# karfly/learnable-triangulation-pytorch

Measured on AMD Instinct MI355X. Metric: multi-view samples/sec (4-view vol-softmax forward), higher is better.
Workload: dtype bf16; 1 GPU; BASELINE config 2: volumetric-softmax forward, 4 views 384x384, 64^3 voxel cube, ResNet-152, random-init weights; per_gpu_batch=64, global_batch=64, parallelism=batch-sharded replicas x1, no data-path collective, hip_graph=True, self_launched=False

## Files before the change

### include/lt_hip.h

```cpp
#ifndef LT_HIP_H
#define LT_HIP_H

#include <stddef.h>
#include <stdint.h>

#ifdef __cplusplus
extern "C" {
#endif

#define LT_ABI_VERSION 1

enum { LT_F32 = 0, LT_BF16 = 1,
       LT_FP8 = 2  };
enum { LT_OK = 0, LT_ERR_INVALID = -1, LT_ERR_UNSUPPORTED = -2, LT_ERR_LAUNCH = -3 };

enum { LT_AGG_SUM = 0, LT_AGG_MAX = 1, LT_AGG_SOFTMAX = 2, LT_AGG_CONF = 3,
       LT_AGG_CONF_NORM = 4  };

enum {
    LT_EPI_RELU_PRE = 1,
    LT_EPI_RELU_POST = 2,
    LT_EPI_STORE_F32 = 4,
    LT_EPI_SIGMOID = 8,
    LT_EPI_RES_F32 = 64,
    LT_BN_FROZEN = 32,
    LT_BN_Y_BF16 = 128,
    LT_ACT_BF16 = 256
};

const char* lt_last_error(void);
int lt_abi_version(void);
int lt_device_info(int* cu_count, int* lds_per_cu, char* arch, int arch_len);

#define LT_CONV_MAX_PHASES 8

typedef struct lt_conv_phase {
    const void* weight;
    const int32_t* taps;
    int32_t ntaps;
    int32_t out_off[3];
    const void* weight_frag;
    int32_t weight_frag_layout;
} lt_conv_phase;

typedef struct lt_conv_desc {
    int32_t dtype;
    int32_t N, D, H, W, Cin;
    int32_t Do, Ho, Wo;
    int32_t stride[3], pad[3];
    int32_t OD, OH, OW;
    int32_t out_stride[3];
    int32_t Cout, ldc;
    int32_t cout_pad, k_pad;
    int32_t nphase;
    int32_t flags;
    int32_t tile;
    int32_t stages;
    lt_conv_phase phase[LT_CONV_MAX_PHASES];
} lt_conv_desc;

int lt_conv_pack_weights(const void* weight, int32_t cout_pad, int32_t k_pad, void* packed, void* stream);
int lt_conv_pack_weights_t32(const void* weight, int32_t cout_pad, int32_t k_pad, int32_t cin, int32_t ntaps, void* packed,
                             void* stream);
int lt_conv_pack_weights32(const void* weight, int32_t cout_pad, int32_t k_pad, void* packed, void* stream);

enum { LT_TILE_AUTO = 0,
       LT_TILE_128x128 = 1, LT_TILE_128x64 = 2, LT_TILE_256x32 = 3, LT_TILE_256x16 = 4, LT_TILE_64x64 = 5,
       LT_TILE2_128x128 = 11, LT_TILE2_128x64 = 12, LT_TILE2_256x32 = 13, LT_TILE2_256x16 = 14, LT_TILE2_64x64 = 15,
       LT_TILE_HALO = 20,
       LT_TILE3_288 = 30,
       LT_TILE_DIRECT = 99  };

int lt_conv_fwd(const lt_conv_desc* desc, const void* x, const float* bias, const float* scale, const float* shift,
                const void* residual, void* y, void* stream);
typedef struct lt_conv_skip {
    const void* x;
    int32_t cin;
    const void* weight_frag;
} lt_conv_skip;
int lt_conv_skip_fwd(const lt_conv_desc* desc, const void* x, const float* bias, const float* scale, const float* shift,
                     const lt_conv_skip* skip, void* y, void* stream);
typedef struct lt_conv_cat2 {
    const void* x;
    int32_t cin, H, W, stride;
} lt_conv_cat2;
int lt_conv_cat2_fwd(const lt_conv_desc* desc, const void* x, const lt_conv_cat2* second, const float* bias, const float* scale, const float* shift,
                     const void* residual, void* y, void* stream);
int lt_conv_cout_pad(int32_t cout);
int32_t lt_conv_chunk_samples(int32_t N, int64_t per_sample);

typedef struct lt_wshape {
    int32_t nd;
    int64_t s[5];
} lt_wshape;
int lt_sel_conv_skip(int32_t dtype, const int32_t x[5], const lt_wshape* w, const int32_t skip_x[5], const lt_wshape* skip_w);
int lt_sel_conv_cat2(int32_t dtype, const int32_t t2[5], const lt_wshape* w_expand, const int32_t x[5], const lt_wshape* w_down, int32_t stride_down);
int lt_sel_splitk_slices(const lt_conv_desc* d, const lt_wshape* w, int32_t transposed);
int lt_sel_bottleneck(int32_t dtype, const int32_t x[5], const lt_wshape w[3], const int32_t strides[3]);
int lt_sel_bottleneck_ds(int32_t dtype, const int32_t x[5], const lt_wshape w[3], const int32_t strides[3], const lt_wshape* w_down, int32_t stride_down);
int lt_sel_expand_reduce(int32_t dtype, const int32_t t2[5], const int32_t res[5], const lt_wshape* w_expand, const lt_wshape* w_reduce);
int lt_sel_stem_pool(int32_t dtype, const int32_t x[5], const lt_wshape* w, int32_t stride, int32_t pad, const int32_t pool[3]);
int lt_sel_pwchain(int32_t dtype, const int32_t x[5], int32_t nlayers, const lt_wshape* w);
int lt_sel_frag_layout(const lt_conv_desc* d, const lt_wshape* w, int32_t transposed, int32_t has_residual);

int lt_maxpool_fwd(int32_t dtype, const void* x, void* y, int32_t N, int32_t D, int32_t H, int32_t W, int32_t C,
                   const int32_t k[3], const int32_t s[3], const int32_t p[3], void* stream);

int lt_global_avgpool(int32_t dtype, const void* x, void* y, int32_t N, int32_t HW, int32_t C, void* stream);

int lt_nchw_to_nhwc(int32_t dtype, const float* x, void* y, int32_t N, int32_t C, int32_t HW, int32_t c_pad, void* stream);
int lt_nhwc_to_nchw_f32(int32_t dtype, const void* x, float* y, int32_t N, int32_t C, int32_t HW, int32_t ld, void* stream);

int lt_splitk_reduce(int32_t dtype, const float* partial, int32_t S, int64_t N, int64_t rows_per_sample, int32_t C, const float* bias,
                     const float* scale, const float* shift, const void* residual, void* y, int32_t flags, void* stream);

int lt_coord_volumes(const float* pos, const float* center, const float* rot, float step, int32_t B, int32_t V,
                     int32_t cmu_transfer, float* coords, void* stream);
int lt_rotate_points(const float* x, const float* rot, float* y, int64_t n, void* stream);

int lt_unproject_fwd(int32_t dtype, const void* feats, const float* proj, const float* coords, const float* conf,
                     void* out, int32_t B, int32_t NV, int32_t C, int32_t h, int32_t w, int32_t v0, int32_t v1,
                     int32_t v2, int32_t agg, void* stream);
int lt_unproject_grid_fwd(int32_t dtype, const void* feats, const float* proj, const float* pos, const float* center, const float* rot,
                          float step, int32_t cmu_transfer, float* coords_out, const float* conf, void* out, int32_t B, int32_t NV,
                          int32_t C, int32_t h, int32_t w, int32_t V, int32_t agg, void* stream);
int lt_unproject_masked_fwd(int32_t dtype, const void* feats, const float* proj, const float* coords, const float* conf, const uint8_t* view_mask,
                            void* out, int32_t B, int32_t NV, int32_t C, int32_t h, int32_t w, int32_t v0, int32_t v1, int32_t v2, int32_t agg,
                            void* stream);
int lt_unproject_grid_masked_fwd(int32_t dtype, const void* feats, const float* proj, const float* pos, const float* center, const float* rot,
                                 float step, int32_t cmu_transfer, float* coords_out, const float* conf, const uint8_t* view_mask, void* out,
                                 int32_t B, int32_t NV, int32_t C, int32_t h, int32_t w, int32_t V, int32_t agg, void* stream);
enum { LT_KIND_MPII = 0, LT_KIND_COCO = 1 };
int lt_cuboid_from_keypoints(const float* keypoints_3d, int32_t B, int32_t J, int32_t kind, double cuboid_side, float* pos, float* center,
                             void* stream);

size_t lt_softargmax3d_workspace(int32_t B, int32_t J, int64_t nvox);
int lt_softargmax3d_fwd(const float* logits, const float* coords, float mult, int32_t softmax, int32_t channels_last,
                        int32_t ld, float* kp, float* probs, int32_t B, int32_t J, int64_t nvox, void* workspace,
                        void* stream);

int lt_softargmax2d_fwd(const float* heatmaps, float mult, int32_t softmax, float* coords, float* probs, int32_t NJ,
                        int32_t h, int32_t w, void* stream);
int lt_softargmax2d_bwd(const float* probs, const float* coords, const float* grad_coords, float mult, int32_t softmax, float* grad_heatmaps,
                        int32_t NJ, int32_t h, int32_t w, void* stream);
int lt_triangulate_dlt_bwd(const float* proj, const float* points, const float* conf, const float* grad_out, float* grad_points, float* grad_conf,
                           int32_t B, int32_t NV, int32_t J, void* stream);

size_t lt_unproject_bwd_workspace(int32_t B, int32_t NV, int32_t C, int32_t v0, int32_t v1, int32_t v2);
int lt_unproject_bwd(int32_t dtype, const void* feats, const float* proj, const float* coords, const float* conf, const float* grad_out,
                     float* grad_feats, float* grad_conf, int32_t B, int32_t NV, int32_t C, int32_t h, int32_t w, int32_t v0, int32_t v1,
                     int32_t v2, int32_t agg, void* workspace, size_t workspace_bytes, void* stream);
int lt_softargmax3d_bwd(const float* probs, const float* coords, const float* kp, const float* grad_kp, const int32_t* gp_idx,
                        const float* gp_val, float multiplier, int32_t softmax, int32_t channels_last, float* grad_logits, int32_t B,
                        int32_t J, int64_t nvox, void* stream);
int lt_softargmax3d_bwd_dense(const float* probs, const float* coords, const float* kp, const float* grad_kp, const int32_t* gp_idx,
                              const float* gp_val, const float* gp_dense, float* workspace_bj, float multiplier, int32_t softmax,
                              int32_t channels_last, float* grad_logits, int32_t B, int32_t J, int64_t nvox, void* stream);
int lt_volumetric_ce_fwd(const float* coords, const float* probs, const float* keypoints_gt, const float* validity, float* terms,
                         int32_t* idx, float* grad_val, int32_t B, int32_t J, int64_t nvox, void* stream);
size_t lt_bn_stats_workspace(int64_t rows, int32_t C);
int lt_bn_stats_fwd(int32_t dtype, const void* x, int64_t rows, int32_t C, float* mean, float* var, float* running_mean,
                    float* running_var, float momentum, void* workspace, void* stream);

int lt_bn_act_fwd(const void* y , const float* mean, const float* var, const float* gamma, const float* beta, const void* residual, void* z,
                  void* z_bf16 , int64_t rows, int32_t C, float eps,
                  int32_t flags, void* stream);
size_t lt_bn_act_bwd_workspace(int64_t rows, int32_t C);
int lt_bn_act_bwd(const void* dz, const void* y , const void* residual, const float* mean, const float* var, const float* gamma, const float* beta,
                  void* dy, void* dy_bf16 , float* dgamma, float* dbeta, void* dres, int32_t accumulate_res,
                  int64_t rows, int32_t C, float eps, int32_t flags, void* workspace, void* stream);
int lt_act_bwd(const void* dz, const void* z, const void* residual, void* dy, void* dres, int32_t accumulate_res, int64_t total, int32_t flags,
               void* stream);
size_t lt_channel_sum_workspace(int64_t rows, int32_t C);
int lt_channel_sum(const float* x, int64_t rows, int32_t C, float* out, int32_t accumulate, void* workspace, void* stream);
int lt_channel_sum_dt(int32_t dtype, const void* x, int64_t rows, int32_t C, float* out, int32_t accumulate, void* workspace, void* stream);
int lt_maxpool_bwd(const float* x, const float* dy, float* dx, int32_t N, int32_t D, int32_t H, int32_t W, int32_t C, const int32_t k[3],
                   const int32_t s[3], const int32_t p[3], void* stream);
int lt_maxpool_bwd_dt(int32_t dtype, const void* x, const void* dy, void* dx, int32_t N, int32_t D, int32_t H, int32_t W, int32_t C, const int32_t k[3],
                      const int32_t s[3], const int32_t p[3], void* stream);
size_t lt_conv_wgrad_workspace(int64_t rows, int32_t cout_pad, int32_t k_pad);
int lt_conv_wgrad(const float* dy, const float* x, const int32_t* taps, float* dw, int32_t N, int32_t D, int32_t H, int32_t W, int32_t Cin, int32_t Do,
                  int32_t Ho, int32_t Wo, const int32_t stride[3], const int32_t pad[3], int32_t Cout, int32_t ldy, int32_t cout_pad, int32_t k_pad,
// ... 26 lines not shown
int lt_quant_fp8_dt(int32_t dtype, const void* x, void* q, int64_t n, const float* amax, float* scale_out, void* stream);
int lt_gather_f32_fp8(const float* src, const int32_t* idx, void* q, int64_t n, const float* amax, float* scale_out, void* stream);
int lt_scale_product(float* dst, int32_t n, const float* a, const float* b, void* stream);
int lt_gather_f32_multi(const void* jobs, int32_t njobs, int32_t total_blocks, void* stream);
int lt_adam_step_multi(const void* jobs, int32_t njobs, int32_t total_blocks, double beta1, double beta2, float eps, float weight_decay, int32_t step,
                       void* stream);
int lt_adam_step(float* param, const float* grad, float* exp_avg, float* exp_avg_sq, int64_t n, float lr, double beta1, double beta2, float eps,
                 float weight_decay, int32_t step, void* stream);

int lt_triangulate_dlt(const float* proj, const float* points, const float* conf, float* out, int32_t B, int32_t NV,
                       int32_t J, void* stream);
int lt_alg_tail_fwd(const float* keypoints_hm, const float* conf_raw, int32_t ld_conf, const float* proj, float scale_x, float scale_y,
                    float* keypoints_2d, float* confidences, float* keypoints_3d, int32_t B, int32_t NV, int32_t J, void* stream);
int lt_alg_tail_masked_fwd(const float* keypoints_hm, const float* conf_raw, int32_t ld_conf, const float* proj, float scale_x, float scale_y,
                           const uint8_t* view_mask, float* keypoints_2d, float* confidences, float* keypoints_3d, int32_t B, int32_t NV,
                           int32_t J, void* stream);

int lt_heatmap_argmax_nchw_f32(const float* heatmaps, int32_t ld, float* heatmaps_nchw, int64_t* indices, int64_t* keypoints,
                               int32_t N, int32_t J, int32_t h, int32_t w, int32_t image_h, int32_t image_w, void* stream);
int lt_triangulate_ransac(const float* proj, const int64_t* points, const int32_t* pairs, int32_t n_iters, double eps, int32_t direct_opt,
                          float* out_kp3d, uint8_t* out_inliers, int32_t B, int32_t NV, int32_t J, void* stream);

int lt_crop_resize_u8(const uint8_t* src, int64_t src_bytes, const int64_t* desc, const int64_t* desc_host, int32_t N, int32_t H, int32_t W,
                      const float* lut, float* out, void* stream);

int lt_undistort_crop_resize_u8(const uint8_t* src, int64_t src_bytes, const int64_t* desc, const int64_t* desc_host, const int16_t* maps,
                                int64_t maps_bytes, int32_t N, int32_t H, int32_t W, const float* lut, float* out, void* stream);

#define LT_PWCHAIN_MAX 3
typedef struct {
    int32_t dtype;
    int32_t nlayers;
    int64_t rows;
    int32_t cin;
    int32_t ldy;
    int32_t cout[LT_PWCHAIN_MAX];
    int32_t k_pad[LT_PWCHAIN_MAX];
    int32_t flags[LT_PWCHAIN_MAX];
    const void* weight[LT_PWCHAIN_MAX];
    const float* bias[LT_PWCHAIN_MAX];
    const float* scale[LT_PWCHAIN_MAX];
    const float* shift[LT_PWCHAIN_MAX];
    int64_t plane;
} lt_pwchain_desc;
int lt_pwchain_fwd(const lt_pwchain_desc* desc, const void* x, void* y, void* stream);

typedef struct {
    int32_t dtype;
    int32_t N, H, W;
    int32_t Cin, Cout;
    const void* weight;
    const float* bias;
    const float* scale;
    const float* shift;
    int32_t x_layout;
} lt_stem_desc;
size_t lt_stem_packed_bytes(void);
int lt_stem_pack_weights(const void* weight, int32_t k_pad, void* packed, void* stream);
int lt_stem_pool_fwd(const lt_stem_desc* desc, const void* x, void* y, void* stream);

typedef struct {
    int32_t dtype;
    int32_t N, H, W;
    int32_t C, P;
    const void* weight[3];
    const float* bias[3];
    const float* scale[3];
    const float* shift[3];
} lt_bneck_desc;
int lt_bottleneck_fwd(const lt_bneck_desc* desc, const void* x, void* y, void* stream);

typedef struct {
    int32_t dtype;
    int32_t N, H, W;
    int32_t Cin, P, C;
    const void* weight[4];
    const float* scale[4];
    const float* shift[4];
} lt_bneck_ds_desc;
int lt_bottleneck_ds_fwd(const lt_bneck_ds_desc* desc, const void* x, void* y, void* stream);

typedef struct {
    int32_t dtype;
    int32_t C, P;
    int64_t M;
    const void* weight[2];
    const float* scale[2];
    const float* shift[2];
    const float* consts;
} lt_xr_desc;
int lt_expand_reduce_fwd(const lt_xr_desc* desc, const void* t2, const void* residual, void* y, void* t1_next, void* stream);

int lt_graph_begin(void* stream);
int lt_graph_end(void* stream, void** graph_exec_out);
int lt_graph_launch(void* graph_exec, void* stream);
int lt_graph_destroy(void* graph_exec);
int lt_event_create(void** ev_out);
int lt_event_record(void* ev, void* stream);
int lt_event_elapsed_ms(void* ev_start, void* ev_stop, float* ms_out);
int lt_event_destroy(void* ev);

typedef struct lt_plan lt_plan;
typedef struct lt_named_tensor {
    const char* name;
    const float* data;
    int32_t ndim;
    int64_t shape[5];
} lt_named_tensor;
typedef struct lt_vol_plan_config {
    int32_t dtype;
    int32_t num_layers;
    int32_t style_caffe;
    int32_t num_joints;
    int32_t B, NV, H, W;
    int32_t volume_size;
    double cuboid_side;
    double volume_multiplier;
    int32_t volume_softmax;
    int32_t aggregation;
    int32_t transfer_cmu_to_human36m;
    int32_t use_graph;
} lt_vol_plan_config;
typedef struct lt_plan_info_t {
    int32_t launches;
    int32_t heatmap_h, heatmap_w;
    double flops;
    int64_t bytes_allocated;
    int32_t n_expand_reduce, n_bottleneck, n_bottleneck_ds, n_conv_cat2, n_conv2d_halo, n_pwchain, n_stem_pool, n_splitk, n_conv_skip;
    int32_t graph_captured;
    const float* logits;
    int32_t logits_planar;
} lt_plan_info_t;
int lt_plan_create_vol(const lt_vol_plan_config* cfg, const lt_named_tensor* weights, int32_t nweights, lt_plan** plan_out);
int lt_plan_forward_vol(lt_plan* plan, const float* images, const double* K_host, const double* R_host, const double* t_host, const double* base_points_host,
                        const double* rot_host, float* keypoints_3d, float* volumes, float* features, float* coord_volumes, float* vol_confidences, void* stream);
enum { LT_MODEL_ALG = 1, LT_MODEL_RANSAC = 2 };
typedef struct lt_alg_plan_config {
    int32_t model;
    int32_t dtype;
    int32_t num_layers;
    int32_t style_caffe;
    int32_t num_joints;
    int32_t B, NV, H, W;
    int32_t use_confidences;
    int32_t heatmap_softmax;
    double heatmap_multiplier;
    int32_t direct_optimization;
    double reprojection_error_epsilon;
    int32_t use_graph;
} lt_alg_plan_config;
int lt_plan_create_alg(const lt_alg_plan_config* cfg, const lt_named_tensor* weights, int32_t nweights, lt_plan** plan_out);
int lt_plan_forward_alg(lt_plan* plan, const float* images, const float* proj, float* keypoints_3d, void* keypoints_2d, float* heatmaps,
                        float* confidences, void* stream);
typedef struct lt_cascade_plan_config {
    lt_alg_plan_config alg;
    lt_vol_plan_config vol;
    int32_t kind;
} lt_cascade_plan_config;
int lt_plan_create_cascade(const lt_cascade_plan_config* cfg, const lt_named_tensor* alg_weights, int32_t n_alg, const lt_named_tensor* vol_weights,
                           int32_t n_vol, lt_plan** plan_out);
int lt_plan_forward_cascade(lt_plan* plan, const float* images, const double* K_host, const double* R_host, const double* t_host, const double* rot_host,
                            float* keypoints_3d, float* alg_keypoints_3d, float* base_points, float* volumes, float* features, float* coord_volumes,
                            float* vol_confidences, void* stream);
int lt_plan_set_view_mask(lt_plan* plan, const uint8_t* mask_host);
int lt_plan_info(const lt_plan* plan, lt_plan_info_t* info);
void lt_plan_destroy(lt_plan* plan);
// ... 6 lines not shown
```

### learnable-triangulation-pytorch_amd/csrc/bneck.hip

```cpp
#include <stdlib.h>

#include <type_traits>

#include "wave_prims.h"

using namespace lt;

namespace {

__device__ uint4 g_zero_page_b[2];

#ifdef LT_BNECK_TRACE
#define LT_BNECK_TRACE_WG 4096
__device__ unsigned long long g_bneck_trace[LT_BNECK_TRACE_WG * 4 * 8];
#define BN_STAMP(k)                                                                                                  \
    do {                                                                                                             \
        if (blockIdx.x < LT_BNECK_TRACE_WG && lane == 0) g_bneck_trace[(blockIdx.x * 4 + wave) * 8 + (k)] = clock64(); \
    } while (0)
#else
#define BN_STAMP(k)
#endif

struct BneckArgs {
    const bf16_t* x;
    bf16_t* y;
    const bf16_t* w1;
    const bf16_t* w2;
    const bf16_t* w3;
    const float* bias[3];
    const float* scale[3];
    const float* shift[3];
    int N, H, W, tiles_x, tiles_y;
};

template <int NK1, int AHEAD, int D>
constexpr int bneck_after(int ks) {
    int total = 0, last = 0;
    for (int k = 0; k < D && k < NK1; ++k) { total += 2; if (k == ks) last = total; }
    for (int k = 0; k < AHEAD && k < NK1; ++k) { total += 3; if (k == ks && total > last) last = total; }
    for (int s = 0; s < ks; ++s) {
        if (s + D < NK1) { total += 2; if (s + D == ks && total > last) last = total; }
        if (s + AHEAD < NK1) { total += 3; if (s + AHEAD == ks && total > last) last = total; }
    }
    return total - last;
}

template <int C, int P, int NSTR, int NHELD>
__global__ __launch_bounds__(256, 2) void bneck_kernel(const BneckArgs a) {
    typedef bf16_t T;
    constexpr int TH = 8, TW = 16, HPI = TW + 2, HROWS = (TH + 2) * HPI;
    constexpr int NPB = 4;
    constexpr int NCB = P / 32, NOB = C / 32, G2 = P / 16, NK1 = C / 32;
    constexpr int RB = 2 * P, NSL = P / 8;
    constexpr int T1_BYTES = HROWS * RB;
    constexpr int STAGE = HROWS * 64;
    constexpr int NT1 = T1_BYTES / STAGE, NST = NT1 + NSTR;
    constexpr int T2_OFF = T1_BYTES;
    constexpr int AHEAD = NST - 1 < NK1 ? NST - 1 : NK1;
    constexpr int NPB1 = NCB == 4 ? 6 : 3, NPB2 = NCB == 4 ? 4 : 2, NOBW = NOB / 4;
    static_assert(NCB == 2 || NCB == 4, "bottleneck width 64 or 128");
    static_assert(T1_BYTES % STAGE == 0, "t1 is a whole number of ring stages");
    static_assert(NPB * 32 * RB <= (NSTR - 1) * STAGE + 192 * 64, "t2 fits behind t1");
    static_assert(NK1 % 2 == 0 && NHELD <= NOBW && NHELD <= 2, "K steps / held residual blocks");
    static_assert(T1_BYTES % 256 == 0 && STAGE % 256 == 0, "the XOR / bank arguments assume 256-byte aligned regions");
    auto fsw = [](int hp) -> int { return NSL == 16 ? (hp & 15) : ((hp >> 1) & 7); };

    extern __shared__ __attribute__((aligned(1024))) unsigned char smem[];
    const unsigned lds0 = (unsigned)(size_t)(lptr_t)smem;
    unsigned long long zp_bits = (unsigned long long)(size_t)g_zero_page_b;
    asm volatile("" : "+s"(zp_bits));
    const void* const zero_page = (const void*)(size_t)zp_bits;

    const int t = threadIdx.x, lane = t & 63;
    const int wave = __builtin_amdgcn_readfirstlane(t >> 6);
    int lin = blockIdx.x;
    {
        const int nb = gridDim.x, q = nb >> 3, r = nb & 7, xcd = lin & 7, j = lin >> 3;
        lin = (xcd < r ? xcd * (q + 1) : r * (q + 1) + (xcd - r) * q) + j;
    }
    const int tpi = a.tiles_x * a.tiles_y;
    const int img = lin / tpi, rem = lin - img * tpi;
    const int ty = rem / a.tiles_x, tx = rem - ty * a.tiles_x;
    const int y0 = ty * TH - 1, x0 = tx * TW - 1;
    const T* __restrict__ x = a.x;

    const int n31 = lane & 31, hk = lane >> 5;
    const int cb = NCB == 4 ? wave : (wave & 1);
    const int whalf = NCB == 4 ? 0 : (wave >> 1);
    const int prr = n31 >> 4, pcc = ((n31 & 15) - 2 * prr) & 15;

    uint4 held[NHELD > 0 ? NHELD : 1][NPB][2];

    float4 cst12, cst3;
    {
        const int l = lane & 31, arr = l >> 3, i4 = l & 7;
        const float* t12 = arr == 0 ? a.scale[0] : arr == 1 ? a.shift[0] : arr == 2 ? a.scale[1] : a.shift[1];
        cst12 = *(const float4*)(t12 + 32 * cb + 4 * i4);
        const int f = (4 * lane) % (NOBW * 64), q = f >> 6, which = (f >> 5) & 1, c = f & 31;
        cst3 = *(const float4*)((which ? a.shift[2] : a.scale[2]) + 32 * (wave + 4 * q) + c);
    }
    auto cget = [&](const float4& tb, int f) -> float {
        const float v = (f & 3) == 0 ? tb.x : (f & 3) == 1 ? tb.y : (f & 3) == 2 ? tb.z : tb.w;
        return __int_as_float(__builtin_amdgcn_readlane(__float_as_int(v), f >> 2));
    };
    auto csel = [&](const float4& tb, int base, int e) -> float {
        const float lo = cget(tb, base + 16 * (e >> 3) + (e & 7)), hi = cget(tb, base + 16 * (e >> 3) + 8 + (e & 7));
        return hk ? hi : lo;
    };

    BN_STAMP(0);
    {
#ifndef LT_BNECK_ABL_SEG128
        const int prow = lane >> 2;
#endif
#ifdef LT_BNECK_ABL_SEG128
        const int prow = lane >> 3;
        const int kvlog = lane & 7;
#elif defined(LT_BNECK_ABL_NOSWZ)
        const int kvlog = lane & 3;
#else
        const int kvlog = (lane & 3) ^ swz64(prow);
#endif
        int dbase[3];
        bool dact[3];
#pragma unroll
        for (int i = 0; i < 3; ++i) {
            const int hp = 16 * (wave + 4 * i) + prow;
            const int hr = hp / HPI, hc = hp - hr * HPI;
            const int iy = y0 + hr, ix = x0 + hc;
            const bool ok = (hp < HROWS) & ((unsigned)iy < (unsigned)a.H) & ((unsigned)ix < (unsigned)a.W);
            dbase[i] = ok ? ((img * a.H + iy) * a.W + ix) * C + kvlog * 8 : -1;
// ... 35 lines not shown
                for (int j = 0; j < 2; ++j)
                    dst[pb][j] = *(const uint4*)((lptr_t)(size_t)(lds0 + stage_base + hpc * 64 + (((2 * j + hk) ^ swz64(hpc)) << 4)));
            }
        };

        f32x16 acc[NPB1];
#pragma unroll
        for (int i = 0; i < NPB1; ++i)
#pragma unroll
            for (int e = 0; e < 16; ++e) acc[i][e] = 0.f;

        static_for<0, DA>([&](auto kc) { loadA(decltype(kc)::value, fa[decltype(kc)::value]); });
#pragma unroll
        for (int s = 0; s < AHEAD; ++s)
            static_for<0, 3>([&](auto ic) { issue_piece(s, s * STAGE, ic); });

        static_for<0, NK1>([&](auto kc) {
            constexpr int ks = decltype(kc)::value, R = ks % NFA;
            constexpr unsigned rbuf = (ks % NST) * STAGE, wbuf = ((ks + AHEAD) % NST) * STAGE;
            wait_vmcnt<bneck_after<NK1, AHEAD, DA>(ks)>();
            asm volatile("s_waitcnt lgkmcnt(0)\n\ts_barrier" ::: "memory");
            frag_ready(fa[R][0]);
            frag_ready(fa[R][1]);
            if constexpr (ks + DA < NK1) loadA(ks + DA, fa[(ks + DA) % NFA]);
            if constexpr (ks + AHEAD < NK1) static_for<0, 3>([&](auto ic) { issue_piece(ks + AHEAD, wbuf, ic); });
            if constexpr (NHELD > 0 && ks < 4) { if (ks == wave) capture(rbuf, held[0]); }
            if constexpr (NHELD > 1 && ks >= 4 && ks < 8) { if (ks == wave + 4) capture(rbuf, held[NHELD > 1 ? 1 : 0]); }
            const unsigned rb = lds0 + rbuf + hb0 * 2048;
#ifndef LT_BNECK_ABL_NOMMA1
            V16 b0[NPB1], b1[NPB1];
#pragma unroll
            for (int i = 0; i < NPB1; ++i) b0[i].u = *(const uint4*)((lptr_t)(size_t)(rb + fo0 + i * 2048));
            __builtin_amdgcn_sched_barrier(0);
#pragma unroll
            for (int i = 0; i < NPB1; ++i) b1[i].u = *(const uint4*)((lptr_t)(size_t)(rb + fo1 + i * 2048));
#pragma unroll
            for (int i = 0; i < NPB1; ++i) acc[i] = __builtin_amdgcn_mfma_f32_32x32x16_bf16(fa[R][0].h, b0[i].h, acc[i], 0, 0, 0);
            __builtin_amdgcn_sched_barrier(0);
#pragma unroll
            for (int i = 0; i < NPB1; ++i) acc[i] = __builtin_amdgcn_mfma_f32_32x32x16_bf16(fa[R][1].h, b1[i].h, acc[i], 0, 0, 0);
            __builtin_amdgcn_sched_barrier(0);
#else
            acc[0][0] += fa[R][0].f[0] + fa[R][1].f[0];
#endif
        });
        asm volatile("s_waitcnt vmcnt(0)\n\ts_waitcnt lgkmcnt(0)\n\ts_barrier" ::: "memory");
        BN_STAMP(1);

        float esc[16], esf[16];
#pragma unroll
        for (int e = 0; e < 16; ++e) {
            esc[e] = csel(cst12, 0, e);
            esf[e] = csel(cst12, 32, e);
        }
        if (a.bias[0]) {
#pragma unroll
            for (int e = 0; e < 16; ++e) esf[e] = a.bias[0][32 * cb + 16 * (e >> 3) + 8 * hk + (e & 7)] * esc[e] + esf[e];
        }
#pragma unroll
        for (int i = 0; i < NPB1; ++i) {
            const int hp = 32 * (hb0 + i) + n31;
            const int hr = hp / HPI, hc = hp - hr * HPI;
            const int iy = y0 + hr, ix = x0 + hc;
            const bool inimg = ((unsigned)iy < (unsigned)a.H) & ((unsigned)ix < (unsigned)a.W);
            if (hp < HROWS) {
#pragma unroll
                for (int q = 0; q < 2; ++q) {
                    unsigned o[4];
#pragma unroll
                    for (int d = 0; d < 4; ++d) {
                        const int e = 8 * q + 2 * d;
                        const float v0 = fmaxf(acc[i][e] * esc[e] + esf[e], 0.f), v1 = fmaxf(acc[i][e + 1] * esc[e + 1] + esf[e + 1], 0.f);
                        o[d] = inimg ? pack_bf16x2(v0, v1) : 0u;
                    }
                    const int slot = (4 * cb + 2 * q + hk) ^ fsw(hp);
                    *(uint4*)((lptr_t)(size_t)(lds0 + hp * RB + slot * 16)) = make_uint4(o[0], o[1], o[2], o[3]);
                }
            }
        }
    }
    __syncthreads();
    BN_STAMP(2);

    constexpr int NU3 = NOBW * G2, WD3 = G2 < 6 ? G2 : 6;
    int poff[NPB];
#pragma unroll
    for (int pb = 0; pb < NPB; ++pb)
        poff[pb] = ((img * a.H + ty * TH + 2 * pb + prr) * a.W + tx * TW + pcc) * C + 8 * hk;
    const T* wl3 = a.w3 + (size_t)lane * 8;
    auto load_w3 = [&](int u) -> V16 {
        const int q = u / G2, g = u - q * G2;
        V16 v;
        v.u = *(const uint4*)(wl3 + ((size_t)g * NOB + wave + 4 * q) * 512);
        return v;
    };
    V16 wf3[WD3 + 1];
    uint4 rq[2][NPB][2];
    auto load_res = [&](int q, uint4 (&dst)[NPB][2]) {
        const int ob = wave + 4 * q;
#pragma unroll
        for (int pb = 0; pb < NPB; ++pb)
#pragma unroll
            for (int j = 0; j < 2; ++j) dst[pb][j] = *(const uint4*)(x + poff[pb] + 32 * ob + 16 * j);
    };

    {
        const int pb0 = NCB == 4 ? 0 : 2 * whalf;
        const int bn = prr * HPI + pcc + 2 * HPI * pb0;
        unsigned am[16];
#pragma unroll
        for (int m = 0; m < 16; ++m) am[m] = lds0 + bn * RB + ((hk ^ fsw(bn + m)) << 4);
        const T* wl = a.w2 + ((size_t)cb * 64 + lane) * 8;
        auto load_w = [&](int u) -> V16 {
            V16 v;
            v.u = *(const uint4*)(wl + (size_t)u * NCB * 512);
            return v;
        };
        constexpr int NU = 9 * G2, WD = 6;
        V16 wf[WD + 1];
#pragma unroll
        for (int u = 0; u < WD; ++u) wf[u] = load_w(u);
        f32x16 acc[NPB2];
#pragma unroll
        for (int i = 0; i < NPB2; ++i)
#pragma unroll
            for (int e = 0; e < 16; ++e) acc[i][e] = 0.f;
        V16 xa[2][NPB2];
        auto load_x = [&](auto uc, V16 (&dst)[NPB2]) {
            constexpr int u = decltype(uc)::value;
            constexpr int tap = u / G2, g = u % G2, dy = tap / 3, dx = tap % 3;
            static_for<0, NPB2>([&](auto ic) {
                constexpr int i = decltype(ic)::value;
                constexpr int TT = dy * HPI + dx + 2 * HPI * i;
                const unsigned ad = am[TT & 15] ^ (g << 5);
                dst[i].u = *(const uint4*)((lptr_t)(size_t)(ad + TT * RB));
            });
        };
        load_x(std::integral_constant<int, 0>{}, xa[0]);
        static_for<0, NU>([&](auto uc) {
            constexpr int u = decltype(uc)::value;
            if constexpr (u + WD < NU) wf[(u + WD) % (WD + 1)] = load_w(u + WD);
            if constexpr (u + 1 < NU) load_x(std::integral_constant<int, u + 1>{}, xa[(u + 1) & 1]);
#pragma unroll
            for (int i = 0; i < NPB2; ++i)
                acc[i] = __builtin_amdgcn_mfma_f32_32x32x16_bf16(wf[u % (WD + 1)].h, xa[u & 1][i].h, acc[i], 0, 0, 0);
            __builtin_amdgcn_sched_barrier(0);
        });
        BN_STAMP(3);
#pragma unroll
        for (int u = 0; u < WD3; ++u) wf3[u] = load_w3(u);
        if constexpr (NHELD < NOBW) load_res(NHELD, rq[0]);
        __builtin_amdgcn_sched_barrier(0);

        float esc[16], esf[16];
#pragma unroll
        for (int e = 0; e < 16; ++e) {
            esc[e] = csel(cst12, 64, e);
            esf[e] = csel(cst12, 96, e);
        }
        if (a.bias[1]) {
#pragma unroll
            for (int e = 0; e < 16; ++e) esf[e] = a.bias[1][32 * cb + 16 * (e >> 3) + 8 * hk + (e & 7)] * esc[e] + esf[e];
        }
#pragma unroll
        for (int i = 0; i < NPB2; ++i) {
            const int px = 32 * (pb0 + i) + n31;
#pragma unroll
            for (int q = 0; q < 2; ++q) {
                unsigned o[4];
#pragma unroll
                for (int d = 0; d < 4; ++d) {
                    const int e = 8 * q + 2 * d;
                    o[d] = pack_bf16x2(fmaxf(acc[i][e] * esc[e] + esf[e], 0.f), fmaxf(acc[i][e + 1] * esc[e + 1] + esf[e + 1], 0.f));
                }
                const int slot = (4 * cb + 2 * q + hk) ^ fsw(n31);
                *(uint4*)((lptr_t)(size_t)(lds0 + T2_OFF + px * RB + slot * 16)) = make_uint4(o[0], o[1], o[2], o[3]);
            }
        }
    }
    __syncthreads();
    BN_STAMP(4);

    {
        const unsigned a2 = lds0 + T2_OFF + n31 * RB + ((hk ^ fsw(n31)) << 4);
        f32x16 acc[NPB];
        static_for<0, NU3>([&](auto uc) {
            constexpr int u = decltype(uc)::value;
            constexpr int q = u / G2, g = u % G2;
            const int ob = wave + 4 * q;
            if constexpr (g == 0) {
#pragma unroll
                for (int pb = 0; pb < NPB; ++pb)
#pragma unroll
                    for (int e = 0; e < 16; ++e) acc[pb][e] = 0.f;
            }
            if constexpr (g == G2 - WD3 && q + 1 < NOBW && q + 1 > NHELD) load_res(q + 1, rq[(q + 1 - NHELD) & 1]);
            if constexpr (u + WD3 < NU3) wf3[(u + WD3) % (WD3 + 1)] = load_w3(u + WD3);
            V16 xb[NPB];
#pragma unroll
            for (int pb = 0; pb < NPB; ++pb) xb[pb].u = *(const uint4*)((lptr_t)(size_t)((a2 ^ (g << 5)) + pb * 32 * RB));
#pragma unroll
            for (int pb = 0; pb < NPB; ++pb)
                acc[pb] = __builtin_amdgcn_mfma_f32_32x32x16_bf16(wf3[u % (WD3 + 1)].h, xb[pb].h, acc[pb], 0, 0, 0);
            __builtin_amdgcn_sched_barrier(0);
            if constexpr (g == G2 - 1) {
#pragma unroll
                for (int j = 0; j < 2; ++j) {
                    float esc[8], esf[8];
#pragma unroll
                    for (int e = 0; e < 8; ++e) {
                        esc[e] = csel(cst3, 64 * q, 8 * j + e);
                        esf[e] = csel(cst3, 64 * q + 32, 8 * j + e);
                    }
                    if (a.bias[2]) {
#pragma unroll
                        for (int e = 0; e < 8; ++e) esf[e] = a.bias[2][32 * ob + 16 * j + 8 * hk + e] * esc[e] + esf[e];
                    }
#pragma unroll
                    for (int pb = 0; pb < NPB; ++pb) {
                        uint4 rv;
                        if constexpr (q < NHELD) rv = held[q < NHELD ? q : 0][pb][j];
                        else rv = rq[(q - NHELD) & 1][pb][j];
                        const unsigned rr[4] = {rv.x, rv.y, rv.z, rv.w};
                        unsigned o[4];
#pragma unroll
                        for (int d = 0; d < 4; ++d) {
                            const int e = 2 * d;
                            const float v0 = fmaxf(acc[pb][8 * j + e] * esc[e] + esf[e] + __uint_as_float(rr[d] << 16), 0.f);
                            const float v1 = fmaxf(acc[pb][8 * j + e + 1] * esc[e + 1] + esf[e + 1] + __uint_as_float(rr[d] & 0xffff0000u), 0.f);
                            o[d] = pack_bf16x2(v0, v1);
                        }
                        *(uint4*)(a.y + poff[pb] + 32 * ob + 16 * j) = make_uint4(o[0], o[1], o[2], o[3]);
                    }
                }
            }
        });
    }
    BN_STAMP(5);
}

template <int C, int P, int NSTR, int NHELD>
int launch_bneck(const BneckArgs& a, hipStream_t s) {
    constexpr int RB = 2 * P;
    constexpr int lds = 180 * RB + (NSTR - 1) * 180 * 64 + 192 * 64;
    static_assert(lds <= 80 * 1024, "two workgroups per CU");
    auto kern = bneck_kernel<C, P, NSTR, NHELD>;
    LT_OPT_IN_LDS(kern, lds);
    const long long nblk = (long long)a.N * a.tiles_x * a.tiles_y;
    hipLaunchKernelGGL(kern, dim3((unsigned)nblk), dim3(256), lds, s, a);
    LT_CHECK_LAUNCH("lt_bottleneck_fwd");
    return LT_OK;
}


struct BneckDsArgs {
    const bf16_t* x;
    bf16_t* y;
    const bf16_t* w1;
    const bf16_t* w2;
    const bf16_t* w3;
    const bf16_t* wd;
    const float* scale[4];
    const float* shift[4];
    int N, H, W, tiles_x, tiles_y;
};

template <int CIN, int P, int C>
__global__ __launch_bounds__(256, 2) void bneck_ds_kernel(const BneckDsArgs a) {
    typedef bf16_t T;
    constexpr int TH = 8, TW = 16, HPI = TW + 2, HROWS = (TH + 2) * HPI;
    constexpr int NPB = 4;
    constexpr int NCB = P / 32, NOB = C / 32, G2 = P / 16, GD = CIN / 16, NK1 = CIN / 32;
    constexpr int RB = 2 * P, NSL = P / 8;
    constexpr int T1_BYTES = HROWS * RB, STAGE = HROWS * 64;
    constexpr int XS_OFF = T1_BYTES, T2_OFF = XS_OFF + NK1 * STAGE;
    constexpr int NPB1 = 3, NPB2 = 2, NOBW = NOB / 4;
    static_assert(CIN == 64 && P == 64 && C == 256, "the first block of ResNet layer1");
    static_assert(NCB == 2 && NSL == 8 && NOBW == 2, "wave roles below");
    static_assert(XS_OFF % 256 == 0 && T2_OFF % 256 == 0, "the XOR / bank arguments assume 256-byte aligned regions");
    auto fsw = [](int hp) -> int { return (hp >> 1) & 7; };

    extern __shared__ __attribute__((aligned(1024))) unsigned char smem[];
    const unsigned lds0 = (unsigned)(size_t)(lptr_t)smem;
    unsigned long long zp_bits = (unsigned long long)(size_t)g_zero_page_b;
    asm volatile("" : "+s"(zp_bits));
    const void* const zero_page = (const void*)(size_t)zp_bits;

    const int t = threadIdx.x, lane = t & 63;
    const int wave = __builtin_amdgcn_readfirstlane(t >> 6);
    int lin = blockIdx.x;
    {
        const int nb = gridDim.x, q = nb >> 3, r = nb & 7, xcd = lin & 7, j = lin >> 3;
        lin = (xcd < r ? xcd * (q + 1) : r * (q + 1) + (xcd - r) * q) + j;
    }
    const int tpi = a.tiles_x * a.tiles_y;
    const int img = lin / tpi, rem = lin - img * tpi;
    const int ty = rem / a.tiles_x, tx = rem - ty * a.tiles_x;
    const int y0 = ty * TH - 1, x0 = tx * TW - 1;
    const T* __restrict__ x = a.x;

    const int n31 = lane & 31, hk = lane >> 5;
    const int cb = wave & 1, whalf = wave >> 1;
    const int prr = n31 >> 4, pcc = ((n31 & 15) - 2 * prr) & 15;

    float4 cst12, cst3;
    {
        const int l = lane & 31, arr = l >> 3, i4 = l & 7;
        const float* t12 = arr == 0 ? a.scale[0] : arr == 1 ? a.shift[0] : arr == 2 ? a.scale[1] : a.shift[1];
        cst12 = *(const float4*)(t12 + 32 * cb + 4 * i4);
        const int f = 4 * lane, q = f >> 7, which = (f >> 5) & 3, c = f & 31;
        const float* t3 = which == 0 ? a.scale[2] : which == 1 ? a.shift[2] : which == 2 ? a.scale[3] : a.shift[3];
        cst3 = *(const float4*)(t3 + 32 * (wave + 4 * q) + c);
    }
    auto cget = [&](const float4& tb, int f) -> float {
        const float v = (f & 3) == 0 ? tb.x : (f & 3) == 1 ? tb.y : (f & 3) == 2 ? tb.z : tb.w;
        return __int_as_float(__builtin_amdgcn_readlane(__float_as_int(v), f >> 2));
    };
    auto csel = [&](const float4& tb, int base, int e) -> float {
        const float lo = cget(tb, base + 16 * (e >> 3) + (e & 7)), hi = cget(tb, base + 16 * (e >> 3) + 8 + (e & 7));
        return hk ? hi : lo;
    };
// ... 205 lines not shown
            if constexpr (k == NUQ - 1) {
#pragma unroll
                for (int j = 0; j < 2; ++j) {
                    float esc[8], esf[8], dsc[8], dsf[8];
#pragma unroll
                    for (int e = 0; e < 8; ++e) {
                        esc[e] = csel(cst3, 128 * q, 8 * j + e);
                        esf[e] = csel(cst3, 128 * q + 32, 8 * j + e);
                        dsc[e] = csel(cst3, 128 * q + 64, 8 * j + e);
                        dsf[e] = csel(cst3, 128 * q + 96, 8 * j + e);
                    }
#pragma unroll
                    for (int pb = 0; pb < NPB; ++pb) {
                        unsigned o[4];
#pragma unroll
                        for (int d = 0; d < 4; ++d) {
                            const int e = 2 * d;
                            const float r0 = accd[pb][8 * j + e] * dsc[e] + dsf[e], r1 = accd[pb][8 * j + e + 1] * dsc[e + 1] + dsf[e + 1];
                            const float v0 = fmaxf(acc[pb][8 * j + e] * esc[e] + esf[e] + r0, 0.f);
                            const float v1 = fmaxf(acc[pb][8 * j + e + 1] * esc[e + 1] + esf[e + 1] + r1, 0.f);
                            o[d] = pack_bf16x2(v0, v1);
                        }
                        *(uint4*)(a.y + poff[pb] + 32 * ob + 16 * j) = make_uint4(o[0], o[1], o[2], o[3]);
                    }
                }
            }
        });
    }
}

int launch_bneck_ds(const BneckDsArgs& a, hipStream_t s) {
    constexpr int lds = 180 * 128 + 2 * 180 * 64 + 128 * 128;
    static_assert(lds <= 80 * 1024, "two workgroups per CU");
    auto kern = bneck_ds_kernel<64, 64, 256>;
    LT_OPT_IN_LDS(kern, lds);
    const long long nblk = (long long)a.N * a.tiles_x * a.tiles_y;
    hipLaunchKernelGGL(kern, dim3((unsigned)nblk), dim3(256), lds, s, a);
    LT_CHECK_LAUNCH("lt_bottleneck_ds_fwd");
    return LT_OK;
}

}

#ifdef LT_BNECK_TRACE
extern "C" int lt_bneck_trace_read(void* host, int nbytes) {
    return (int)hipMemcpyFromSymbol(host, HIP_SYMBOL(g_bneck_trace), nbytes, 0, hipMemcpyDeviceToHost);
}
#endif

extern "C" int lt_bottleneck_fwd(const lt_bneck_desc* d, const void* x, void* y, void* stream) {
    LT_REQUIRE(d && x && y, LT_ERR_INVALID, "lt_bottleneck_fwd: null argument");
    LT_REQUIRE(x != y, LT_ERR_INVALID, "lt_bottleneck_fwd: in-place is not possible (neighbouring tiles read each other's halo)");
    LT_REQUIRE(d->dtype == LT_BF16, LT_ERR_UNSUPPORTED, "lt_bottleneck_fwd: bf16 only");
    LT_REQUIRE((d->C == 256 && d->P == 64) || (d->C == 512 && d->P == 128), LT_ERR_UNSUPPORTED,
               "lt_bottleneck_fwd: widths %d / %d (256 / 64 and 512 / 128: the identity blocks of ResNet layer1 / layer2)", d->C, d->P);
    LT_REQUIRE(d->N > 0 && d->H > 0 && d->W > 0 && d->H % 8 == 0 && d->W % 16 == 0, LT_ERR_UNSUPPORTED,
               "lt_bottleneck_fwd: map %d x %d (8 x 16 pixel tiles)", d->H, d->W);
    LT_REQUIRE((long long)d->N * d->H * d->W * d->C < (1ll << 31), LT_ERR_UNSUPPORTED, "lt_bottleneck_fwd: 32-bit element offsets");
    BneckArgs a;
    a.x = (const bf16_t*)x;
    a.y = (bf16_t*)y;
    a.w1 = (const bf16_t*)d->weight[0];
    a.w2 = (const bf16_t*)d->weight[1];
    a.w3 = (const bf16_t*)d->weight[2];
    for (int i = 0; i < 3; ++i) {
        LT_REQUIRE(d->weight[i] && d->scale[i] && d->shift[i], LT_ERR_INVALID, "lt_bottleneck_fwd: layer %d: null weight / scale / shift", i);
        a.bias[i] = d->bias[i];
        a.scale[i] = d->scale[i];
        a.shift[i] = d->shift[i];
    }
    a.N = d->N; a.H = d->H; a.W = d->W;
    a.tiles_x = d->W / 16; a.tiles_y = d->H / 8;
    hipStream_t s = (hipStream_t)stream;
#ifndef LT_BNECK_HELD64
#define LT_BNECK_HELD64 2
#endif
#ifndef LT_BNECK_HELD128
#define LT_BNECK_HELD128 1
#endif
    if (d->P == 64) return launch_bneck<256, 64, 4, LT_BNECK_HELD64>(a, s);
    return launch_bneck<512, 128, 3, LT_BNECK_HELD128>(a, s);
}

extern "C" int lt_bottleneck_ds_fwd(const lt_bneck_ds_desc* d, const void* x, void* y, void* stream) {
    LT_REQUIRE(d && x && y, LT_ERR_INVALID, "lt_bottleneck_ds_fwd: null argument");
    LT_REQUIRE(x != y, LT_ERR_INVALID, "lt_bottleneck_ds_fwd: in-place is not possible");
    LT_REQUIRE(d->dtype == LT_BF16, LT_ERR_UNSUPPORTED, "lt_bottleneck_ds_fwd: bf16 only");
    LT_REQUIRE(d->Cin == 64 && d->P == 64 && d->C == 256, LT_ERR_UNSUPPORTED,
               "lt_bottleneck_ds_fwd: widths %d -> %d -> %d (64 -> 64 -> 256: the first block of ResNet layer1)", d->Cin, d->P, d->C);
    LT_REQUIRE(d->N > 0 && d->H > 0 && d->W > 0 && d->H % 8 == 0 && d->W % 16 == 0, LT_ERR_UNSUPPORTED,
               "lt_bottleneck_ds_fwd: map %d x %d (8 x 16 pixel tiles)", d->H, d->W);
    LT_REQUIRE((long long)d->N * d->H * d->W * d->C < (1ll << 31), LT_ERR_UNSUPPORTED, "lt_bottleneck_ds_fwd: 32-bit element offsets");
    BneckDsArgs a;
    a.x = (const bf16_t*)x;
    a.y = (bf16_t*)y;
    for (int i = 0; i < 4; ++i) {
        LT_REQUIRE(d->weight[i] && d->scale[i] && d->shift[i], LT_ERR_INVALID, "lt_bottleneck_ds_fwd: layer %d: null weight / scale / shift", i);
        a.scale[i] = d->scale[i];
        a.shift[i] = d->shift[i];
    }
    a.w1 = (const bf16_t*)d->weight[0];
    a.w2 = (const bf16_t*)d->weight[1];
    a.w3 = (const bf16_t*)d->weight[2];
    a.wd = (const bf16_t*)d->weight[3];
    a.N = d->N; a.H = d->H; a.W = d->W;
    a.tiles_x = d->W / 16; a.tiles_y = d->H / 8;
    return launch_bneck_ds(a, (hipStream_t)stream);
}
```

### learnable-triangulation-pytorch_amd/csrc/plan.hip

```cpp
#include <math.h>
#include <stdlib.h>
#include <string.h>

#include <array>
#include <deque>
#include <functional>
#include <map>
#include <string>
#include <unordered_map>
#include <vector>

#include "lt_common.h"

using namespace lt;

namespace {

#define PL_TRY(call)                   \
    do {                               \
        const int rc_ = (call);        \
        if (rc_ != LT_OK) return rc_;  \
    } while (0)
#define PL_HIP(call)                                                        \
    do {                                                                    \
// ... 142 lines not shown
        const int o = (dims[i] - 1) * 2 - 2 * pd[i] + ks[i] + output_padding;
        LT_REQUIRE(o == 2 * dims[i], LT_ERR_UNSUPPORTED, "plan: a transposed convolution must exactly double the size (k = 4, p = 1 / k = 2, p = 0)");
        outs[i] = o;
    }
    const int cp = cout_pad_of(cout);
    struct DimPhase { int phi; std::vector<std::pair<int, int>> taps; };
    auto dim_phases = [&](int i) {
        std::vector<DimPhase> res;
        if (!nd3 && i == 0) { res.push_back({0, {{0, 0}}}); return res; }
        for (int phi = 0; phi < 2; ++phi) {
            DimPhase dp; dp.phi = phi;
            for (int kk = 0; kk < ks[i]; ++kk)
                if (floormod(phi + pd[i] - kk, 2) == 0) dp.taps.push_back({kk, floordiv(phi + pd[i] - kk, 2)});
            res.push_back(dp);
        }
        return res;
    };
    const int64_t ktot = (int64_t)kd * kh * kw;
    struct Raw { std::vector<std::pair<std::vector<float>, int>> dummy; };
    std::vector<PhaseSpec> phases;
    std::vector<std::vector<int>> phase_k;
    int ntaps_max = 0;
    for (const DimPhase& A : dim_phases(0))
        for (const DimPhase& Bp : dim_phases(1))
            for (const DimPhase& Cp : dim_phases(2)) {
                PhaseSpec ph; std::vector<int> kidx;
                for (auto& ta : A.taps)
                    for (auto& tb : Bp.taps)
                        for (auto& tc : Cp.taps) {
                            const int da = ta.second, db = tb.second, dc = tc.second;
                            ph.taps.push_back(da); ph.taps.push_back(db); ph.taps.push_back(dc); ph.taps.push_back(((da * Hh + db) * W + dc) * cin);
                            kidx.push_back((ta.first * kh + tb.first) * kw + tc.first);
                        }
                if (kidx.empty()) { ph.taps = {0, 0, 0, 0}; kidx.push_back(-1); }
                ph.ntaps = (int)kidx.size();
                ph.off[0] = A.phi; ph.off[1] = Bp.phi; ph.off[2] = Cp.phi;
                if (ph.ntaps > ntaps_max) ntaps_max = ph.ntaps;
                phases.push_back(ph); phase_k.push_back(kidx);
            }
    const int K = ntaps_max * cin, k_pad = (K + kstep - 1) / kstep * kstep;
    for (size_t p = 0; p < phases.size(); ++p) {
        PhaseSpec& ph = phases[p];
        ph.w.assign((size_t)cp * k_pad, 0.f);
        for (int t = 0; t < ph.ntaps; ++t) {
            const int kt = phase_k[p][t];
            if (kt < 0) continue;
            for (int ci = 0; ci < cin; ++ci)
                for (int co = 0; co < cout; ++co) ph.w[(size_t)co * k_pad + (size_t)t * cin + ci] = w.d[((int64_t)ci * cout + co) * ktot + kt];
        }
    }
    LT_REQUIRE((int)phases.size() <= LT_CONV_MAX_PHASES, LT_ERR_UNSUPPORTED, "plan: %d phases", (int)phases.size());
    sp.Cin = cin; sp.Do = D; sp.Ho = Hh; sp.Wo = W; sp.OD = outs[0]; sp.OH = outs[1]; sp.OW = outs[2];
    for (int i = 0; i < 3; ++i) { sp.st[i] = 1; sp.pd[i] = 0; }
    sp.ostr[0] = nd3 ? 2 : 1; sp.ostr[1] = 2; sp.ostr[2] = 2;
    sp.Cout = cout; sp.cout_pad = cp; sp.k_pad = k_pad;
    fold_bn(cout, bias, bn, cp, sp.bias, sp.scale, sp.shift);
    sp.ph = std::move(phases);
    return LT_OK;
}

}

struct lt_plan {
    lt_vol_plan_config cfg;
    int model = 0;
    lt_alg_plan_config acfg = {};
    const char* who = "lt_plan_create_vol";
    int dtype = LT_F32, es = 4;
    std::unordered_map<std::string, const lt_named_tensor*> sd;
    std::vector<void*> allocs;
    std::map<std::pair<size_t, int>, std::vector<char*>> pool;
    size_t bytes_alloc = 0;
    double flops = 0;
    typedef std::function<int(hipStream_t)> Op;
    std::vector<Op> ops;
    int npre = 0, ntail = 0;
    std::deque<lt_conv_desc> conv_descs;
    std::deque<lt_conv_skip> skip_descs;
    std::deque<lt_conv_cat2> cat2_descs;
    std::deque<lt_pwchain_desc> pw_descs;
    std::deque<lt_stem_desc> stem_descs;
    std::deque<lt_bneck_desc> bneck_descs;
    std::deque<lt_bneck_ds_desc> bneck_ds_descs;
    std::deque<lt_xr_desc> xr_descs;
    hipGraphExec_t graph = nullptr;
    bool captured = false;
    hipStream_t own_stream = nullptr; hipEvent_t own_ev[2] = {nullptr, nullptr};
    const float* cur_images = nullptr;
    float* out_kp = nullptr; float* out_probs = nullptr; float* out_feats = nullptr;
    const float* cur_proj = nullptr; void* out_kp2d = nullptr; float* out_hm = nullptr; float* out_conf = nullptr;
    float* geo_dev = nullptr; StagingRing geo; size_t n_geo = 0, o_pos = 0, o_cen = 0, o_rot = 0;
    Act feats, vol, logits, volc;
    float* coords = nullptr; float* kp = nullptr; float* probs = nullptr; void* sa_ws = nullptr;
    Act algc;
    float* hm_nchw = nullptr; float* kp_hm = nullptr; int64_t* kp_i64 = nullptr;
    int hm_h = 0, hm_w = 0;
    lt_plan* sub_alg = nullptr; lt_plan* sub_vol = nullptr; int kind = 0;
    float* cproj_dev = nullptr; StagingRing cproj; float* ckp_alg = nullptr;
    bool masked = false, ran = false, mask_dirty = false;
    std::vector<uint8_t> mask_cur;
    const uint8_t* mask_dev = nullptr; size_t o_mask = 0;
    uint8_t* amask_dev = nullptr; StagingRing amask;
    int n_xr = 0, n_bneck = 0, n_bneck_ds = 0, n_cat2 = 0, n_halo2d = 0, n_pwchain = 0, n_stem = 0, n_splitk = 0, n_conv_skip = 0;

    ~lt_plan() {
        if (graph) (void)hipGraphExecDestroy(graph);
        if (own_stream) (void)hipStreamDestroy(own_stream);
        for (int i = 0; i < 2; ++i) if (own_ev[i]) (void)hipEventDestroy(own_ev[i]);
        for (void* p : allocs) (void)hipFree(p);
        delete sub_alg;
        delete sub_vol;
    }

    int dev_alloc(size_t bytes, void** out) {
        void* p = nullptr;
        PL_HIP(hipMalloc(&p, bytes ? bytes : 16));
        allocs.push_back(p);
        bytes_alloc += bytes;
        *out = p;
        return LT_OK;
    }
    int alloc(int n, int d, int h, int w, int c, int esz, Act& a) {
        a = Act(); a.n = n; a.d = d; a.h = h; a.w = w; a.c = c; a.es = esz;
        auto it = pool.find({a.bytes(), esz});
        if (it != pool.end() && !it->second.empty()) { a.p = it->second.back(); it->second.pop_back(); return LT_OK; }
        void* p; PL_TRY(dev_alloc(a.bytes(), &p)); a.p = (char*)p;
        return LT_OK;
    }
    void release(const Act& a) { if (a.p && a.pooled) pool[{a.bytes(), a.es}].push_back(a.p); }
    int upload(const void* host, size_t bytes, void** out) {
        PL_TRY(dev_alloc(bytes, out));
        PL_HIP(hipMemcpy(*out, host, bytes, hipMemcpyHostToDevice));
        return LT_OK;
    }
    int upload_f32(const std::vector<float>& v, const float** out) { void* p; PL_TRY(upload(v.data(), v.size() * 4, &p)); *out = (const float*)p; return LT_OK; }
    int upload_w(const std::vector<float>& v, const void** out) {
        if (es == 4) { void* p; PL_TRY(upload(v.data(), v.size() * 4, &p)); *out = p; return LT_OK; }
        std::vector<unsigned short> h(v.size());
        for (size_t i = 0; i < v.size(); ++i) h[i] = bf16_rne(v[i]);
        void* p; PL_TRY(upload(h.data(), h.size() * 2, &p)); *out = p;
        return LT_OK;
    }
    int upload_i32(const std::vector<int32_t>& v, const int32_t** out) { void* p; PL_TRY(upload(v.data(), v.size() * 4, &p)); *out = (const int32_t*)p; return LT_OK; }

    int get(const std::string& name, WT& w, int nd_expect = 0) {
        auto it = sd.find(name);
        LT_REQUIRE(it != sd.end(), LT_ERR_INVALID, "%s: state dict has no '%s'", who, name.c_str());
        const lt_named_tensor* t = it->second;
        LT_REQUIRE(t->data && t->ndim >= 1 && t->ndim <= 5 && (!nd_expect || t->ndim == nd_expect), LT_ERR_INVALID, "%s: '%s' has %d dimensions", who, name.c_str(), t->ndim);
        w.d = t->data; w.nd = t->ndim;
        for (int i = 0; i < t->ndim; ++i) w.s[i] = t->shape[i];
        return LT_OK;
    }
    bool has(const std::string& name) const { return sd.find(name) != sd.end(); }
    int get_vec(const std::string& name, int n, const float** out) {
        WT w; PL_TRY(get(name, w));
        LT_REQUIRE(w.numel() == n, LT_ERR_INVALID, "%s: '%s' has %lld elements, expected %d", who, name.c_str(), (long long)w.numel(), n);
        *out = w.d;
        return LT_OK;
    }
    int get_bn(const std::string& prefix, int c, BN& bn) {
        PL_TRY(get_vec(prefix + ".weight", c, &bn.g)); PL_TRY(get_vec(prefix + ".bias", c, &bn.b));
        PL_TRY(get_vec(prefix + ".running_mean", c, &bn.m)); PL_TRY(get_vec(prefix + ".running_var", c, &bn.v));
        return LT_OK;
    }

// ... 167 lines not shown
        flops += 2.0 * N * Ho * Wo * Cc * kp;
        const lt_conv_desc* dp = &d; const lt_conv_cat2* cp = &c2;
        const void* xp = t2.p; void* yp = y.p;
        ops.push_back([=](hipStream_t s) { return lt_conv_cat2_fwd(dp, xp, cp, bi, nullptr, sh, nullptr, yp, s); });
        ++n_cat2;
        return LT_OK;
    }

    struct PwLayer { WT w; const float* bias; const BN* bn; bool relu; };
    int pwchain(const Act& x, const std::vector<PwLayer>& L, Act& y) {
        pw_descs.emplace_back();
        lt_pwchain_desc& d = pw_descs.back();
        memset(&d, 0, sizeof(d));
        d.dtype = dtype; d.nlayers = (int)L.size(); d.rows = (long long)x.n * x.d * x.h * x.w; d.cin = 32;
        int shape[5] = {x.n, x.d, x.h, x.w, x.c};
        int cout_last = 0;
        for (size_t i = 0; i < L.size(); ++i) {
            const bool last = i + 1 == L.size();
            const int fl = (L[i].relu ? LT_EPI_RELU_POST : 0) | (last ? LT_EPI_STORE_F32 : 0);
            ConvSpec sp; PL_TRY(make_conv_spec(L[i].w, L[i].bias, L[i].bn, shape, 1, 0, es, false, fl, 0, sp));
            if (sp.cout_pad < 32) { sp.ph[0].w.resize((size_t)32 * sp.k_pad, 0.f); sp.bias.resize(32, 0.f); sp.scale.resize(32, 0.f); sp.shift.resize(32, 0.f); }
            const void* wdev; PL_TRY(upload_w(sp.ph[0].w, &wdev));
            const float *bi, *sc, *sh;
            PL_TRY(upload_f32(sp.bias, &bi)); PL_TRY(upload_f32(sp.scale, &sc)); PL_TRY(upload_f32(sp.shift, &sh));
            d.cout[i] = sp.Cout; d.k_pad[i] = sp.k_pad; d.flags[i] = fl; d.weight[i] = wdev; d.bias[i] = bi; d.scale[i] = sc; d.shift[i] = sh;
            flops += 2.0 * d.rows * sp.Cout * L[i].w.s[1];
            shape[4] = sp.Cout; cout_last = sp.Cout;
        }
        d.ldy = cout_last;
        const long long vox = (long long)x.d * x.h * x.w;
        const bool planar = vox % 64 == 0;
        if (planar) d.plane = vox;
        PL_TRY(alloc(x.n, x.d, x.h, x.w, cout_last, 4, y));
        y.planar = planar; y.pooled = !planar;
        const lt_pwchain_desc* dp = &d; const void* xp = x.p; void* yp = y.p;
        ops.push_back([=](hipStream_t s) { return lt_pwchain_fwd(dp, xp, yp, s); });
        ++n_pwchain;
        return LT_OK;
    }

    int maxpool(const Act& x, int k, int s, int p, int nd, Act& y) {
        int32_t kk[3] = {nd == 2 ? 1 : k, k, k}, ss[3] = {nd == 2 ? 1 : s, s, s}, pp[3] = {nd == 2 ? 0 : p, p, p};
        const int od = (x.d + 2 * pp[0] - kk[0]) / ss[0] + 1, oh = (x.h + 2 * pp[1] - kk[1]) / ss[1] + 1, ow = (x.w + 2 * pp[2] - kk[2]) / ss[2] + 1;
        PL_TRY(alloc(x.n, od, oh, ow, x.c, x.es, y));
        const int dt = dtype; const Act xa = x; void* yp = y.p;
        std::vector<int32_t> a = {kk[0], kk[1], kk[2], ss[0], ss[1], ss[2], pp[0], pp[1], pp[2]};
        ops.push_back([=](hipStream_t st) { return lt_maxpool_fwd(dt, xa.p, yp, xa.n, xa.d, xa.h, xa.w, xa.c, a.data(), a.data() + 3, a.data() + 6, st); });
        return LT_OK;
    }

    int global_avgpool(const Act& x, Act& y) {
        PL_TRY(alloc(1, 1, 1, x.n, x.c, x.es, y));
        const int dt = dtype; const Act xa = x; void* yp = y.p;
        ops.push_back([=](hipStream_t st) { return lt_global_avgpool(dt, xa.p, yp, xa.n, xa.d * xa.h * xa.w, xa.c, st); });
        return LT_OK;
    }

    int pack_block_layer(const WT& w, const BN& bn, const int in[5], int pad, int fl, const void** wfr, const float** sc, const float** sh, ConvSpec& sp) {
        PL_TRY(make_conv_spec(w, nullptr, &bn, in, 1, pad, es, false, fl, 0, sp));
        LT_REQUIRE(sp.cout_pad == sp.Cout && sp.k_pad == sp.ph[0].ntaps * sp.Cin, LT_ERR_INVALID, "plan: fused block layer padding (%d / %d)", sp.cout_pad, sp.k_pad);
        const void* wdev; PL_TRY(upload_w(sp.ph[0].w, &wdev));
        PL_TRY(pack_frag(wdev, (size_t)sp.cout_pad * sp.k_pad, 2, sp.cout_pad, sp.k_pad, sp.Cin, sp.ph[0].ntaps, wfr));
        PL_TRY(upload_f32(sp.scale, sc)); PL_TRY(upload_f32(sp.shift, sh));
        flops += 2.0 * in[0] * in[2] * in[3] * sp.Cout * sp.ph[0].ntaps * sp.Cin;
        return LT_OK;
    }
    int bottleneck(const Act& x, const WT w[3], const BN bn[3], Act& y) {
        PL_TRY(alloc(x.n, 1, x.h, x.w, x.c, es, y));
        bneck_descs.emplace_back();
        lt_bneck_desc& d = bneck_descs.back();
        memset(&d, 0, sizeof(d));
        d.dtype = dtype; d.N = x.n; d.H = x.h; d.W = x.w; d.C = x.c; d.P = (int)w[0].s[0];
        int shape[5] = {x.n, 1, x.h, x.w, x.c};
        for (int i = 0; i < 3; ++i) {
            ConvSpec sp;
            PL_TRY(pack_block_layer(w[i], bn[i], shape, i == 1 ? 1 : 0, LT_EPI_RELU_POST, &d.weight[i], &d.scale[i], &d.shift[i], sp));
            shape[4] = sp.Cout;
        }
        const lt_bneck_desc* dp = &d; const void* xp = x.p; void* yp = y.p;
        ops.push_back([=](hipStream_t s) { return lt_bottleneck_fwd(dp, xp, yp, s); });
        ++n_bneck;
        return LT_OK;
    }
    int bottleneck_ds(const Act& x, const WT w[3], const BN bn[3], const WT& wd, const BN& bnd, Act& y) {
        const int Cc = (int)w[2].s[0];
        PL_TRY(alloc(x.n, 1, x.h, x.w, Cc, es, y));
        bneck_ds_descs.emplace_back();
        lt_bneck_ds_desc& d = bneck_ds_descs.back();
        memset(&d, 0, sizeof(d));
        d.dtype = dtype; d.N = x.n; d.H = x.h; d.W = x.w; d.Cin = x.c; d.P = (int)w[0].s[0]; d.C = Cc;
        int shape[5] = {x.n, 1, x.h, x.w, x.c};
        for (int i = 0; i < 3; ++i) {
            ConvSpec sp;
            PL_TRY(pack_block_layer(w[i], bn[i], shape, i == 1 ? 1 : 0, LT_EPI_RELU_POST, &d.weight[i], &d.scale[i], &d.shift[i], sp));
            shape[4] = sp.Cout;
        }
        const int xs[5] = {x.n, 1, x.h, x.w, x.c};
        ConvSpec sp;
        PL_TRY(pack_block_layer(wd, bnd, xs, 0, 0, &d.weight[3], &d.scale[3], &d.shift[3], sp));
        const lt_bneck_ds_desc* dp = &d; const void* xp = x.p; void* yp = y.p;
        ops.push_back([=](hipStream_t s) { return lt_bottleneck_ds_fwd(dp, xp, yp, s); });
        ++n_bneck_ds;
        return LT_OK;
    }
    int expand_reduce(const Act& t2, const Act& res, const WT& we, const BN& bne, const WT& wr, const BN& bnr, Act& y, Act& t1) {
        const int N = t2.n, Hh = t2.h, W = t2.w, P = t2.c, Cc = res.c;
        PL_TRY(alloc(N, 1, Hh, W, Cc, es, y));
        PL_TRY(alloc(N, 1, Hh, W, P, es, t1));
        xr_descs.emplace_back();
        lt_xr_desc& d = xr_descs.back();
        memset(&d, 0, sizeof(d));
        d.dtype = dtype; d.C = Cc; d.P = P; d.M = (long long)N * Hh * W;
        const int s2[5] = {t2.n, 1, Hh, W, P}, sr[5] = {res.n, 1, Hh, W, Cc};
        ConvSpec s3, s1;
        PL_TRY(pack_block_layer(we, bne, s2, 0, LT_EPI_RELU_POST, &d.weight[0], &d.scale[0], &d.shift[0], s3));
        PL_TRY(pack_block_layer(wr, bnr, sr, 0, LT_EPI_RELU_POST, &d.weight[1], &d.scale[1], &d.shift[1], s1));
        std::vector<float> packed;
        packed.insert(packed.end(), s3.scale.begin(), s3.scale.end()); packed.insert(packed.end(), s3.shift.begin(), s3.shift.end());
        packed.insert(packed.end(), s1.scale.begin(), s1.scale.end()); packed.insert(packed.end(), s1.shift.begin(), s1.shift.end());
        PL_TRY(upload_f32(packed, &d.consts));
        const lt_xr_desc* dp = &d; const void* a = t2.p; const void* r = res.p; void* yp = y.p; void* tp = t1.p;
        ops.push_back([=](hipStream_t s) { return lt_expand_reduce_fwd(dp, a, r, yp, tp, s); });
        ++n_xr;
        return LT_OK;
    }
    int stem_pool(int N, int Hh, int W, const WT& w, const BN& bn, Act& y) {
        const int in[5] = {N, 1, Hh, W, 8};
        ConvSpec sp;
        PL_TRY(make_conv_spec(w, nullptr, &bn, in, 2, 3, es, false, LT_EPI_RELU_POST, 0, sp));
        const int Hp = (sp.Ho - 1) / 2 + 1, Wp = (sp.Wo - 1) / 2 + 1;
        PL_TRY(alloc(N, 1, Hp, Wp, 64, es, y));
        const void* wdev; PL_TRY(upload_w(sp.ph[0].w, &wdev));
        void* wpk; PL_TRY(dev_alloc(lt_stem_packed_bytes(), &wpk));
        PL_TRY(lt_stem_pack_weights(wdev, sp.k_pad, wpk, nullptr));
        PL_HIP(hipStreamSynchronize(nullptr));
        stem_descs.emplace_back();
        lt_stem_desc& d = stem_descs.back();
        memset(&d, 0, sizeof(d));
        d.dtype = dtype; d.N = N; d.H = Hh; d.W = W; d.Cin = 3; d.Cout = 64; d.weight = wpk; d.x_layout = 1;
        PL_TRY(upload_f32(sp.bias, &d.bias)); PL_TRY(upload_f32(sp.scale, &d.scale)); PL_TRY(upload_f32(sp.shift, &d.shift));
        flops += 2.0 * N * sp.Ho * sp.Wo * 64 * 49 * w.s[1];
        const lt_stem_desc* dp = &d; void* yp = y.p; lt_plan* self = this;
        LT_REQUIRE(ops.empty(), LT_ERR_INVALID, "plan: an op reading the caller's tensor must be the first of the plan");
        ops.push_back([=](hipStream_t s) { return lt_stem_pool_fwd(dp, self->cur_images, yp, s); });
        npre = 1;
        ++n_stem;
        return LT_OK;
    }

    struct Block {
        bool bottleneck; int nconv; WT w[3]; BN bn[3]; int strides[3]; bool has_ds; WT wd; BN bnd; int sds;
        bool identity_bottleneck() const { return bottleneck && !has_ds && strides[0] == 1 && strides[1] == 1 && strides[2] == 1; }
    };
    int load_block(const std::string& pre, bool bott, bool caffe, int stride, bool ds, Block& b) {
        b.bottleneck = bott; b.nconv = bott ? 3 : 2; b.has_ds = ds; b.sds = stride;
        if (bott) { b.strides[0] = caffe ? stride : 1; b.strides[1] = caffe ? 1 : stride; b.strides[2] = 1; }
        else { b.strides[0] = stride; b.strides[1] = 1; b.strides[2] = 1; }
        for (int i = 0; i < b.nconv; ++i) {
            PL_TRY(get(pre + ".conv" + std::to_string(i + 1) + ".weight", b.w[i], 4));
            PL_TRY(get_bn(pre + ".bn" + std::to_string(i + 1), (int)b.w[i].s[0], b.bn[i]));
        }
        if (ds) { PL_TRY(get(pre + ".downsample.0.weight", b.wd, 4)); PL_TRY(get_bn(pre + ".downsample.1", (int)b.wd.s[0], b.bnd)); }
        return LT_OK;
    }
    int record_block(const Block& b, const Act& x, const Act* t1_in, const Block* nxt, Act& y, Act& t1n) {
        t1n = Act();
        const lt_wshape w3[3] = {wshape(b.w[0]), wshape(b.w[1]), wshape(b.w[2])}, wd = wshape(b.wd);
        if (b.bottleneck && !b.has_ds && !t1_in && !nxt && lt_sel_bottleneck(dtype, dims(x).data(), w3, b.strides)) return bottleneck(x, b.w, b.bn, y);
        if (b.bottleneck && b.has_ds && !t1_in && !nxt && lt_sel_bottleneck_ds(dtype, dims(x).data(), w3, b.strides, &wd, b.sds))
            return bottleneck_ds(x, b.w, b.bn, b.wd, b.bnd, y);
        if (t1_in || nxt) {
            Act t1, t2;
            ConvOpt o;
            if (t1_in) t1 = *t1_in;
            else { o = ConvOpt(); o.bn = &b.bn[0]; o.relu = true; PL_TRY(conv(x, b.w[0], o, t1)); }
            o = ConvOpt(); o.bn = &b.bn[1]; o.relu = true; o.pad = 1; PL_TRY(conv(t1, b.w[1], o, t2));
            release(t1);
            const lt_wshape wr = nxt ? wshape(nxt->w[0]) : lt_wshape{};
            if (nxt && lt_sel_expand_reduce(dtype, dims(t2).data(), dims(x).data(), &w3[2], &wr)) {
                PL_TRY(expand_reduce(t2, x, b.w[2], b.bn[2], nxt->w[0], nxt->bn[0], y, t1n));
                release(t2);
                return LT_OK;
            }
            o = ConvOpt(); o.bn = &b.bn[2]; o.relu = true; o.residual = &x; PL_TRY(conv(t2, b.w[2], o, y));
            release(t2);
            return LT_OK;
        }
        if (b.bottleneck && b.has_ds) {
            const int Ho = (x.h - 1) / b.sds + 1, Wo = (x.w - 1) / b.sds + 1;
            const int t2s[5] = {x.n, 1, Ho, Wo, (int)b.w[2].s[1]};
            if (lt_sel_conv_cat2(dtype, t2s, &w3[2], dims(x).data(), &wd, b.sds)) {
                Act t1, t2; ConvOpt o;
                o.bn = &b.bn[0]; o.relu = true; o.stride = b.strides[0]; PL_TRY(conv(x, b.w[0], o, t1));
                o = ConvOpt(); o.bn = &b.bn[1]; o.relu = true; o.stride = b.strides[1]; o.pad = 1; PL_TRY(conv(t1, b.w[1], o, t2));
                release(t1);
                PL_TRY(conv_cat2(t2, b.w[2], b.bn[2], x, b.wd, b.bnd, b.sds, y));
                release(t2);
                return LT_OK;
            }
        }
        Act res = x; bool own_res = false;
        if (b.has_ds) { ConvOpt o; o.bn = &b.bnd; o.stride = b.sds; PL_TRY(conv(x, b.wd, o, res)); own_res = true; }
        Act cur = x;
        for (int i = 0; i < b.nconv; ++i) {
            const bool last = i + 1 == b.nconv;
            ConvOpt o; o.bn = &b.bn[i]; o.relu = true; o.stride = b.strides[i]; o.pad = (int)b.w[i].s[2] / 2; o.residual = last ? &res : nullptr;
            Act z; PL_TRY(conv(cur, b.w[i], o, z));
            if (cur.p != x.p) release(cur);
            cur = z;
        }
        if (own_res) release(res);
        y = cur;
        return LT_OK;
    }

    int record_gap_head(const std::string& pre, const Act& x, Act& out) {
        WT w0, w4; const float *b0, *b4; BN bn1, bn5;
        PL_TRY(get(pre + ".features.0.weight", w0, 4)); PL_TRY(get_vec(pre + ".features.0.bias", (int)w0.s[0], &b0)); PL_TRY(get_bn(pre + ".features.1", (int)w0.s[0], bn1));
        PL_TRY(get(pre + ".features.4.weight", w4, 4)); PL_TRY(get_vec(pre + ".features.4.bias", (int)w4.s[0], &b4)); PL_TRY(get_bn(pre + ".features.5", (int)w4.s[0], bn5));
        Act y, p, g;
        ConvOpt o; o.bias = b0; o.bn = &bn1; o.pad = 1; o.relu = true; PL_TRY(conv(x, w0, o, y));
        PL_TRY(maxpool(y, 2, 2, 0, 2, p)); release(y);
        o = ConvOpt(); o.bias = b4; o.bn = &bn5; o.pad = 1; o.relu = true; PL_TRY(conv(p, w4, o, y)); release(p);
        PL_TRY(maxpool(y, 2, 2, 0, 2, p)); release(y);
        PL_TRY(global_avgpool(p, g)); release(p);
        Act cur = g;
        for (int i = 0; i < 3; ++i) {
            WT lw; const float* lb;
            PL_TRY(get(pre + ".head." + std::to_string(2 * i) + ".weight", lw, 2));
            PL_TRY(get_vec(pre + ".head." + std::to_string(2 * i) + ".bias", (int)lw.s[0], &lb));
            lw.nd = 4; lw.s[2] = 1; lw.s[3] = 1;
            ConvOpt lo; lo.bias = lb; lo.relu = i < 2; lo.sigmoid = i == 2; lo.out_f32 = i == 2;
            Act z; PL_TRY(conv(cur, lw, lo, z)); release(cur);
            cur = z;
        }
        out = cur;
        return LT_OK;
    }

    int record_backbone(int N, int Hh, int W, int num_layers, bool caffe, const char* conf_head, bool want_heatmaps, Act& feats256, Act& conf, Act& heatmaps) {
        int nb[4]; bool bott;
        switch (num_layers) {
            case 18: bott = false; nb[0] = 2; nb[1] = 2; nb[2] = 2; nb[3] = 2; break;
            case 34: bott = false; nb[0] = 3; nb[1] = 4; nb[2] = 6; nb[3] = 3; break;
            case 50: bott = true; nb[0] = 3; nb[1] = 4; nb[2] = 6; nb[3] = 3; break;
            case 101: bott = true; nb[0] = 3; nb[1] = 4; nb[2] = 23; nb[3] = 3; break;
            case 152: bott = true; nb[0] = 3; nb[1] = 8; nb[2] = 36; nb[3] = 3; break;
            default: set_error("%s: num_layers %d (18 / 34 / 50 / 101 / 152)", who, num_layers); return LT_ERR_INVALID;
        }
        if (caffe) bott = true;
        const int exp = bott ? 4 : 1;
        WT w1; BN bn1;
        PL_TRY(get("backbone.conv1.weight", w1, 4)); PL_TRY(get_bn("backbone.bn1", 64, bn1));
        Act y;
        const int32_t stem_in[5] = {N, 1, Hh, W, 8}, pool[3] = {3, 2, 1};
        const lt_wshape ws1 = wshape(w1);
        if (w1.s[1] == 3 && lt_sel_stem_pool(dtype, stem_in, &ws1, 2, 3, pool)) PL_TRY(stem_pool(N, Hh, W, w1, bn1, y));
        else {
            const int cpad = 16 / es;
            Act xin; PL_TRY(alloc(N, 1, Hh, W, cpad, es, xin)); xin.pooled = false;
            const int dt = dtype; lt_plan* self = this; void* xp = xin.p;
            ops.push_back([=](hipStream_t s) { return lt_nchw_to_nhwc(dt, self->cur_images, xp, N, 3, Hh * W, cpad, s); });
            npre = 1;
            ConvOpt o; o.bn = &bn1; o.stride = 2; o.pad = 3; o.relu = true;
            Act c1; PL_TRY(conv(xin, w1, o, c1));
            PL_TRY(maxpool(c1, 3, 2, 1, 2, y)); release(c1);
        }
        int inplanes = 64;
        const int planes_of[4] = {64, 128, 256, 512};
        for (int li = 0; li < 4; ++li) {
            const int planes = planes_of[li], stride = li == 0 ? 1 : 2;
            std::vector<Block> blocks(nb[li]);
            for (int bi = 0; bi < nb[li]; ++bi) {
                const int st = bi == 0 ? stride : 1;
                const bool ds = bi == 0 && (st != 1 || inplanes != planes * exp);
                PL_TRY(load_block("backbone.layer" + std::to_string(li + 1) + "." + std::to_string(bi), bott, caffe, st, ds, blocks[bi]));
                inplanes = planes * exp;
            }
            Act t1; bool have_t1 = false;
            for (int bi = 0; bi < nb[li]; ++bi) {
                const Block& blk = blocks[bi];
                const Block* nxt = bi + 1 < nb[li] ? &blocks[bi + 1] : nullptr;
                const bool chain = nxt && blk.identity_bottleneck() && nxt->identity_bottleneck() && dtype == LT_BF16 && blk.w[2].s[0] == 1024 && blk.w[2].s[1] == 256 &&
                                   nxt->w[0].s[0] == 256 && nxt->w[0].s[1] == 1024;
                Act z, t1n;
                if (chain) PL_TRY(record_block(blk, y, have_t1 ? &t1 : nullptr, nxt, z, t1n));
                else if (have_t1) PL_TRY(record_block(blk, y, &t1, nullptr, z, t1n));
                else PL_TRY(record_block(blk, y, nullptr, nullptr, z, t1n));
                release(y);
                y = z; t1 = t1n; have_t1 = !t1n.null();
            }
        }
        conf = Act();
        if (conf_head) PL_TRY(record_gap_head(conf_head, y, conf));
        for (int i = 0; i < 3; ++i) {
            WT dw; BN dbn;
            PL_TRY(get("backbone.deconv_layers." + std::to_string(3 * i) + ".weight", dw, 4));
            PL_TRY(get_bn("backbone.deconv_layers." + std::to_string(3 * i + 1), (int)dw.s[1], dbn));
            const float* db = nullptr;
            if (has("backbone.deconv_layers." + std::to_string(3 * i) + ".bias")) PL_TRY(get_vec("backbone.deconv_layers." + std::to_string(3 * i) + ".bias", (int)dw.s[1], &db));
            LT_REQUIRE(dw.s[2] == 4 && dw.s[3] == 4, LT_ERR_UNSUPPORTED, "%s: only the 4x4 stride-2 deconvolution of the reference configs", who);
            ConvOpt o; o.bias = db; o.bn = &dbn; o.stride = 2; o.pad = 1; o.transposed = true; o.relu = true;
            Act z; PL_TRY(conv(y, dw, o, z)); release(y);
            y = z;
        }
        feats256 = y;
        heatmaps = Act();
        if (want_heatmaps) {
            WT fw; const float* fb;
            PL_TRY(get("backbone.final_layer.weight", fw, 4)); PL_TRY(get_vec("backbone.final_layer.bias", (int)fw.s[0], &fb));
            ConvOpt o; o.bias = fb; o.pad = fw.s[2] == 3 ? 1 : 0; o.out_f32 = true;
            PL_TRY(conv(y, fw, o, heatmaps));
        }
        return LT_OK;
    }

    struct C3 { WT w; const float* b = nullptr; BN bn; bool has_bn = false; };
    int load_c3(const std::string& conv, const std::string& bnname, bool transposed, C3& c) {
        PL_TRY(get(conv + ".weight", c.w, 5));
        const int cout = (int)(transposed ? c.w.s[1] : c.w.s[0]);
        PL_TRY(get_vec(conv + ".bias", cout, &c.b));
        if (!bnname.empty()) { PL_TRY(get_bn(bnname, cout, c.bn)); c.has_bn = true; }
        return LT_OK;
    }
    int res3d(const std::string& pre, const Act& x, Act& out) {
        C3 c0, c3, sk;
        PL_TRY(load_c3(pre + ".res_branch.0", pre + ".res_branch.1", false, c0));
        PL_TRY(load_c3(pre + ".res_branch.3", pre + ".res_branch.4", false, c3));
        const bool has_skip = has(pre + ".skip_con.0.weight");
        if (has_skip) PL_TRY(load_c3(pre + ".skip_con.0", pre + ".skip_con.1", false, sk));
        const int mid[5] = {x.n, x.d, x.h, x.w, (int)c0.w.s[0]};
        Act y, z;
        const lt_wshape w3 = wshape(c3.w), wsk = has_skip ? wshape(sk.w) : lt_wshape{};
        if (has_skip && lt_sel_conv_skip(dtype, mid, &w3, dims(x).data(), &wsk)) {
            ConvOpt o; o.bias = c0.b; o.bn = &c0.bn; o.pad = 1; o.relu = true; PL_TRY(conv(x, c0.w, o, y));
            o = ConvOpt(); o.bias = c3.b; o.bn = &c3.bn; o.pad = 1; o.relu = true; o.skip_x = &x; o.skip_w = &sk.w; o.skip_bias = sk.b; o.skip_bn = &sk.bn;
            PL_TRY(conv(y, c3.w, o, z)); release(y);
            out = z;
            return LT_OK;
        }
        Act skip = x; bool own = false;
        if (has_skip) { ConvOpt o; o.bias = sk.b; o.bn = &sk.bn; PL_TRY(conv(x, sk.w, o, skip)); own = true; }
        ConvOpt o; o.bias = c0.b; o.bn = &c0.bn; o.pad = 1; o.relu = true; PL_TRY(conv(x, c0.w, o, y));
        o = ConvOpt(); o.bias = c3.b; o.bn = &c3.bn; o.pad = 1; o.relu = true; o.residual = &skip; PL_TRY(conv(y, c3.w, o, z));
        release(y);
        if (own) release(skip);
        out = z;
        return LT_OK;
    }
    int record_v2v(const Act& vol_in, Act& logits_out) {
        const std::string V = "volume_net.";
        Act x = vol_in, y;
        {
            C3 c; PL_TRY(load_c3(V + "front_layers.0.block.0", V + "front_layers.0.block.1", false, c));
            ConvOpt o; o.bias = c.b; o.bn = &c.bn; o.pad = (int)(c.w.s[2] - 1) / 2; o.relu = true;
            PL_TRY(conv(x, c.w, o, y)); release(x); x = y;
            for (int i = 1; i <= 3; ++i) { PL_TRY(res3d(V + "front_layers." + std::to_string(i), x, y)); release(x); x = y; }
        }
        {
            const std::string E = V + "encoder_decoder.";
            Act skips[5];
            for (int lvl = 1; lvl <= 5; ++lvl) {
                PL_TRY(res3d(E + "skip_res" + std::to_string(lvl), x, skips[lvl - 1]));
                Act p; PL_TRY(maxpool(x, 2, 2, 0, 3, p)); release(x);
                PL_TRY(res3d(E + "encoder_res" + std::to_string(lvl), p, x)); release(p);
// ... 509 lines not shown
```

### learnable-triangulation-pytorch_amd/csrc/select.hip

```cpp
#include "conv_common.h"

using namespace lt;

namespace {

bool wshape_is(const lt_wshape* w, int nd, int64_t s0, int64_t s1, int64_t s2, int64_t s3, int64_t s4 = 0) {
    const int64_t s[5] = {s0, s1, s2, s3, s4};
    if (w->nd != nd) return false;
    for (int i = 0; i < nd; ++i)
        if (w->s[i] != s[i]) return false;
    return true;
}

bool pointwise(const lt_wshape* w) {
    for (int i = 2; i < w->nd; ++i)
        if (w->s[i] != 1) return false;
    return true;
}

}

extern "C" int lt_sel_conv_skip(int32_t dtype, const int32_t x[5], const lt_wshape* w, const int32_t skip_x[5], const lt_wshape* skip_w) {
    if (dtype != LT_BF16 || env_on("LT_NO_CONV_SKIP") || env_on("LT_HALO_NO_COL") || env_on("LT_HALO_NO_PERSIST") || env_on("LT_CONV_NO_HALO")) return 0;
    if (!wshape_is(w, 5, 32, 32, 3, 3, 3) || !wshape_is(skip_w, 5, 32, 16, 1, 1, 1)) return 0;
    const int N = x[0], D = x[1], H = x[2], W = x[3];
    if (x[4] != 32 || skip_x[0] != N || skip_x[1] != D || skip_x[2] != H || skip_x[3] != W || skip_x[4] != 16) return 0;
    const int nc = lt_conv_chunk_samples(N, (long long)D * H * W * 32);
    if (nc < 1) return 0;
    return halo_col_fits(nc, D, H, W) && halo_col_fits(N - (N - 1) / nc * nc, D, H, W);
}

extern "C" int lt_sel_conv_cat2(int32_t dtype, const int32_t t2[5], const lt_wshape* we, const int32_t x[5], const lt_wshape* wd, int32_t s) {
    if (dtype != LT_BF16 || env_on("LT_NO_CONV_CAT2") || env_on("LT_CONV_NO_V7") || env_on("LT_CONV_NO_V3")) return 0;
    const int N = t2[0], Ho = t2[2], Wo = t2[3], P = t2[4];
    if (t2[1] != 1 || we->nd != 4 || wd->nd != 4 || !pointwise(we) || !pointwise(wd)) return 0;
    const long long Cc = we->s[0], Cin2 = wd->s[1];
    if (we->s[1] != P || wd->s[0] != Cc || (s != 1 && s != 2) || x[0] != N || x[1] != 1 || x[2] != Ho * s || x[3] != Wo * s || x[4] != Cin2) return 0;
    if (P % 32 || Cin2 % 32 || (P + Cin2) % 64 || Cc % 256 || (P & (P - 1))) return 0;
    const long long tiles = (((long long)N * Ho * Wo + 287) / 288) * (Cc / 256);
    if (tiles < 200 && !env_on("LT_CAT2_ANY_SIZE")) return 0;
    return (long long)N * Ho * Wo * Cc < (1ll << 31) && (long long)N * x[2] * x[3] * Cin2 < (1ll << 31);
}

extern "C" int lt_sel_splitk_slices(const lt_conv_desc* d, const lt_wshape* w, int32_t transposed) {
    if (d->dtype != LT_BF16 || transposed || (d->flags & (LT_EPI_STORE_F32 | LT_EPI_SIGMOID)) || env_on("LT_CONV_NO_SPLITK")) return 1;
    if (w->nd != 5 || w->s[2] != 3 || w->s[3] != 3 || w->s[4] != 3) return 1;
    for (int i = 0; i < 3; ++i)
        if (d->stride[i] != 1 || d->pad[i] != 1) return 1;
    if (d->Cin < 128 || d->Cin % 64 || d->Cout % 4 || d->Cout != d->cout_pad || d->D * d->H * d->W > 512) return 1;
    const long long rows = (long long)d->N * d->Do * d->Ho * d->Wo;
    const int bm = rows >= 8192 ? 128 : 64;
    const long long tiles = ((rows + bm - 1) / bm) * (d->cout_pad / bm);
    const long long S = 256 / tiles;
    return S > 8 ? 8 : S < 1 ? 1 : (int)S;
}

extern "C" int lt_sel_bottleneck(int32_t dtype, const int32_t x[5], const lt_wshape w[3], const int32_t strides[3]) {
    if (dtype != LT_BF16 || env_on("LT_NO_BNECK")) return 0;
    if (x[1] != 1 || strides[0] != 1 || strides[1] != 1 || strides[2] != 1) return 0;
    const int C = x[4];
    const int64_t P = w[0].s[0];
    if (!((C == 256 && P == 64) || (C == 512 && P == 128))) return 0;
    if (!wshape_is(&w[0], 4, P, C, 1, 1) || !wshape_is(&w[1], 4, P, P, 3, 3) || !wshape_is(&w[2], 4, C, P, 1, 1)) return 0;
    return x[2] % 8 == 0 && x[3] % 16 == 0 && (long long)x[0] * x[2] * x[3] * C < (1ll << 31);
}

extern "C" int lt_sel_bottleneck_ds(int32_t dtype, const int32_t x[5], const lt_wshape w[3], const int32_t strides[3], const lt_wshape* wd, int32_t sd) {
    if (dtype != LT_BF16 || env_on("LT_NO_BNECK") || env_on("LT_NO_BNECK_DS")) return 0;
    if (x[1] != 1 || strides[0] != 1 || strides[1] != 1 || strides[2] != 1 || sd != 1) return 0;
    if (x[4] != 64 || !wshape_is(&w[0], 4, 64, 64, 1, 1) || !wshape_is(&w[1], 4, 64, 64, 3, 3) || !wshape_is(&w[2], 4, 256, 64, 1, 1) ||
        !wshape_is(wd, 4, 256, 64, 1, 1))
        return 0;
    return x[2] % 8 == 0 && x[3] % 16 == 0 && (long long)x[0] * x[2] * x[3] * 256 < (1ll << 31);
}

extern "C" int lt_sel_expand_reduce(int32_t dtype, const int32_t t2[5], const int32_t res[5], const lt_wshape* we, const lt_wshape* wr) {
    if (dtype != LT_BF16 || env_on("LT_NO_XR")) return 0;
    if (t2[1] != 1 || res[1] != 1 || t2[0] != res[0] || t2[2] != res[2] || t2[3] != res[3] || res[4] != 1024 || t2[4] != 256) return 0;
    if ((long long)t2[0] * t2[2] * t2[3] < 36 * 96 && !env_on("LT_XR_ANY_SIZE")) return 0;
    return wshape_is(we, 4, 1024, 256, 1, 1) && wshape_is(wr, 4, 256, 1024, 1, 1);
}

extern "C" int lt_sel_stem_pool(int32_t dtype, const int32_t x[5], const lt_wshape* w, int32_t stride, int32_t pad, const int32_t pool[3]) {
    return dtype == LT_BF16 && x[1] == 1 && x[4] == 8 && w->nd == 4 && w->s[2] == 7 && w->s[3] == 7 && w->s[0] == 64 && w->s[1] <= 8 && stride == 2 &&
           pad == 3 && pool[0] == 3 && pool[1] == 2 && pool[2] == 1;
}

extern "C" int lt_sel_pwchain(int32_t dtype, const int32_t x[5], int32_t nlayers, const lt_wshape* w) {
    if (dtype != LT_BF16 || nlayers < 1 || nlayers > LT_PWCHAIN_MAX || x[4] != 32) return 0;
    if ((long long)x[0] * x[1] * x[2] * x[3] % 64) return 0;
    int64_t cin = 32;
    for (int i = 0; i < nlayers; ++i) {
        if (!pointwise(&w[i]) || w[i].s[1] != cin || w[i].s[0] > 32 || (i + 1 < nlayers && w[i].s[0] != 32)) return 0;
        cin = w[i].s[0];
    }
    return 1;
}

extern "C" int lt_sel_frag_layout(const lt_conv_desc* d, const lt_wshape* w, int32_t transposed, int32_t has_residual) {
    if (d->dtype != LT_BF16) return 0;
    const bool w3x3 = !transposed && wshape_is(w, 4, 256, 256, 3, 3) && d->W == 24;
    const bool w4x4t = transposed && wshape_is(w, 4, 256, 256, 4, 4) && !env_on("LT_DECONV_NO_H2D");
    if ((w3x3 || w4x4t) && d->tile == LT_TILE_AUTO && !has_residual && !env_on("LT_CONV_NO_H2D") && !env_on("LT_CONV_V1") &&
        ((long long)d->N * (d->H / 8) * (d->W / 24) >= 60 || env_on("LT_H2D_ANY_SIZE")) && halo2d_fits(conv_args_of(*d), d->cout_pad, d->nphase))
        return 2;
    if (d->cout_pad % 256 == 0 && d->k_pad % 64 == 0) {
        const bool short_pw = pointwise(w) && d->k_pad <= 256 && !transposed;
        return !env_on("LT_CONV_NO_V7") && !short_pw ? 3 : 1;
    }
    const bool wreg = wshape_is(w, 5, 64, 64, 3, 3, 3) || wshape_is(w, 5, 64, 32, 3, 3, 3) || wshape_is(w, 5, 128, 128, 3, 3, 3) || wshape_is(w, 5, 32, 16, 3, 3, 3);
    if (transposed || !wreg || d->Cin != w->s[1]) return 0;
    for (int i = 0; i < 3; ++i)
        if (d->stride[i] != 1 || d->pad[i] != 1) return 0;
    return 2;
}
```

### learnable-triangulation-pytorch_amd/lt_engine.py

```python
import ctypes as C
from collections import OrderedDict
from dataclasses import dataclass, field
from typing import List, Optional, Tuple

import numpy as np
import torch
import torch.nn as nn

import lt_hip as H

BN_EPS = 1e-5


def cout_pad_of(cout):
    if cout <= 16:
        return 16
    if cout <= 32:
        return 32
    if cout <= 64:
        return 64
    return (cout + 127) // 128 * 128


def conv_chunk_samples(N, per_sample):
# ... 98 lines not shown
        k_pad = (K + kstep - 1) // kstep * kstep
        wk = w.permute(0, 2, 3, 4, 1).reshape(cout, K)
        taps = [(a, b, c, ((a * Hh + b) * W + c) * cin_buf) for a in range(kd) for b in range(kh) for c in range(kw)]
        bi, sc, sh = fold_bn(cout, bias, bn, cp)
        spec = ConvSpec(N, D, Hh, W, cin_buf, Do, Ho, Wo, st, pd, Do, Ho, Wo, (1, 1, 1), cout, cp, k_pad, flags, bi, sc, sh)
        spec.phases.append(ConvPhaseSpec(_pad_k(wk, cp, k_pad), torch.tensor(taps, dtype=torch.int32).reshape(-1, 4), (0, 0, 0)))
        return spec
    cin, cout, kd, kh, kw = w.shape
    assert cin == cin_buf, "transposed conv input may not be channel padded"
    nd3 = weight.dim() == 5
    assert all(s == 2 for s in (st if nd3 else st[1:])), "only stride-2 transposed convolutions"
    ks = (kd, kh, kw)
    dims = (D, Hh, W)
    outs = []
    for i in range(3):
        if not nd3 and i == 0:
            outs.append(1)
        else:
            o = (dims[i] - 1) * 2 - 2 * pd[i] + ks[i] + output_padding
            assert o == 2 * dims[i], "transposed conv must exactly double the size (k=4,p=1 / k=2,p=0; with output_padding=1: k=3,p=1 / k=1,p=0 -- the input gradients of the stride-2 convolutions)"
            outs.append(o)
    cp = cout_pad_of(cout)

    def dim_phases(i):
        if not nd3 and i == 0:
            return [(0, [(0, 0)])]
        res = []
        for phi in (0, 1):
            res.append((phi, [(kk, (phi + pd[i] - kk) // 2) for kk in range(ks[i]) if (phi + pd[i] - kk) % 2 == 0]))
        return res

    phase_list = []
    ntaps_max = 0
    for pa, ta in dim_phases(0):
        for pb, tb in dim_phases(1):
            for pc, tc in dim_phases(2):
                taps, cols = [], []
                for (ka, da) in ta:
                    for (kb, db) in tb:
                        for (kc, dc) in tc:
                            taps.append((da, db, dc, ((da * Hh + db) * W + dc) * cin))
                            cols.append(w[:, :, ka, kb, kc].t())
                if not taps:
                    taps, cols = [(0, 0, 0, 0)], [torch.zeros(cout, cin)]
                wk = torch.cat(cols, dim=1)
                phase_list.append((wk, taps, (pa, pb, pc)))
                ntaps_max = max(ntaps_max, len(taps))
    K = ntaps_max * cin
    k_pad = (K + kstep - 1) // kstep * kstep
    bi, sc, sh = fold_bn(cout, bias, bn, cp)
    ostr = (2 if nd3 else 1, 2, 2)
    spec = ConvSpec(N, D, Hh, W, cin, D, Hh, W, (1, 1, 1), (0, 0, 0), outs[0], outs[1], outs[2], ostr, cout, cp, k_pad, flags, bi, sc, sh)
    for wk, taps, off in phase_list:
        spec.phases.append(ConvPhaseSpec(_pad_k(wk, cp, k_pad), torch.tensor(taps, dtype=torch.int32).reshape(-1, 4), off))
    assert len(spec.phases) <= H.MAX_PHASES
    return spec


def stage_images(x, act, stream):
    N, Cc, Hh, W = x.shape
    H.check(H.lib().lt_nchw_to_nhwc(H.dtype_code(act.t.dtype), x.data_ptr(), act.t.data_ptr(), N, Cc, Hh * W, act.t.shape[-1], stream), "lt_nchw_to_nhwc")


class Act:
    __slots__ = ("t", "pooled")

    def __init__(self, t):
        self.t = t
        self.pooled = True

    @property
    def shape(self):
        return tuple(self.t.shape)


class Recorder:

    dtype = torch.float32
    live_weights = False

    def _declines(self, *a, **k):
        return False

    can_conv_skip = can_conv_cat2 = can_chain_pointwise = can_bottleneck = can_bottleneck_ds = can_expand_reduce = can_stem_pool = _declines


class PlanBuilder(Recorder):

    def __init__(self, device, dtype, tile_override=0, dry_run=False, stages=0):
        self.device = torch.device(device)
        self.dry_run = dry_run
        if self.device.type != "cuda" and not dry_run:
            raise RuntimeError("liblt_hip plans run on the GPU only (device=%s); there is no CPU fallback" % device)
        self.lib = None if dry_run else H.lib()
        self.dtype = dtype
        self.code = H.dtype_code(dtype)
        self.out_dtype = torch.bfloat16 if dtype == torch.float8_e4m3fn else dtype
        self.ops = []
        self.keep = []
        self.pool = {}
        self.tile_override = tile_override
        self.stages = stages
        self.live_weights = False
        self.live_frag = False
        self.flops = 0
        self.bytes_alloc = 0
        self.ntail = 0
        self.npre = 0

    def alloc(self, shape, dtype=None):
        dtype = dtype or self.dtype
        n = int(np.prod(shape)) * esize(dtype)
        lst = self.pool.get((n, dtype))
        if lst:
            t = lst.pop().view(*shape)
        else:
            t = torch.empty(shape, dtype=dtype, device=self.device)
            self.bytes_alloc += n
        self.keep.append(t)
        return Act(t)

    def release(self, act):
        if act is None or not act.pooled:
            return
        t = act.t
        n = t.numel() * t.element_size()
        self.pool.setdefault((n, t.dtype), []).append(t.reshape(-1))

    def const(self, t, dtype=None):
        t = t.to(device=self.device, dtype=dtype or t.dtype).contiguous()
        self.keep.append(t)
        return t

    def _add(self, fn, kind="op", label="", flops=0, nbytes=0, info=None):
        meta = {"kind": kind, "label": label, "flops": flops, "bytes": nbytes}
        if self.dry_run:
            meta["info"] = info or {}
        self.last_info = info or {}
        self.ops.append((fn, meta))

    def _fusable(self):
        return not (self.live_weights or self.tile_override)

    def can_conv_skip(self, x_shape, weight, skip_shape, skip_weight):
        if not self._fusable():
            return False
        return bool(H.lib().lt_sel_conv_skip(self.code, H.dims(x_shape), H.wshape(weight), H.dims(skip_shape), H.wshape(skip_weight)))

    def _desc(self, spec):
        d = H.ConvDesc()
        d.dtype = self.code
        d.N, d.D, d.H, d.W, d.Cin = spec.N, spec.D, spec.H, spec.W, spec.Cin
        d.Do, d.Ho, d.Wo = spec.Do, spec.Ho, spec.Wo
        d.stride = H.i3(spec.stride); d.pad = H.i3(spec.pad)
        d.OD, d.OH, d.OW = spec.OD, spec.OH, spec.OW
        d.out_stride = H.i3(spec.out_stride)
        d.Cout, d.ldc, d.cout_pad, d.k_pad = spec.Cout, spec.Cout, spec.cout_pad, spec.k_pad
        d.nphase, d.flags, d.tile, d.stages = len(spec.phases), spec.flags, self.tile_override, self.stages
        for i, ph in enumerate(spec.phases):
            d.phase[i].ntaps = ph.taps.shape[0]; d.phase[i].out_off = H.i3(ph.out_off)
        return d

    def frag_layout(self, spec, weight, transposed, residual):
        if self.live_weights and not self.live_frag:
            return 0
        return H.lib().lt_sel_frag_layout(self._desc(spec), H.wshape(weight), int(transposed), int(residual))

# ... 193 lines not shown
        assert self.can_chain_pointwise(x, layers)
        N, D, Hh, W, _ = x.shape
        d = H.PwChainDesc()
        d.dtype, d.nlayers, d.rows, d.cin = self.code, len(layers), N * D * Hh * W, 32
        specs = []
        shape = x.shape
        flops = 0
        for i, (w, bias, bn, relu) in enumerate(layers):
            last = i + 1 == len(layers)
            flags = (H.EPI_RELU_POST if relu else 0) | (H.EPI_STORE_F32 if last else 0)
            spec = make_conv_spec(w, bias, bn, shape, 1, 0, self.dtype, False, flags)
            specs.append(spec)
            rows = lambda t: t if t.shape[0] >= 32 else torch.cat([t, t.new_zeros((32 - t.shape[0],) + tuple(t.shape[1:]))])
            wdev = self.const(rows(spec.phases[0].weight), self.dtype)
            bi, sc, sh = self.const(rows(spec.bias)), self.const(rows(spec.scale)), self.const(rows(spec.shift))
            d.cout[i], d.k_pad[i], d.flags[i] = spec.Cout, spec.k_pad, flags
            d.weight[i], d.bias[i], d.scale[i], d.shift[i] = wdev.data_ptr(), bi.data_ptr(), sc.data_ptr(), sh.data_ptr()
            flops += 2 * d.rows * spec.Cout * w.shape[1]
            shape = (N, D, Hh, W, spec.Cout)
        d.ldy = specs[-1].Cout
        planar = bool(planar) and (D * Hh * W) % 64 == 0
        if planar:
            d.plane = D * Hh * W
            y = Act(self.alloc((N, shape[-1], D, Hh, W), torch.float32).t.permute(0, 2, 3, 4, 1))
            y.pooled = False
        else:
            y = self.alloc(shape, torch.float32)
        self.keep.append(x.t)
        self.keep.append(d)
        self.flops += flops
        label = "pwchain " + "->".join(str(c) for c in [32] + [sp.Cout for sp in specs]) + " @" + "x".join(str(v) for v in (N, D, Hh, W))
        nbytes = x.t.numel() * x.t.element_size() + y.t.numel() * 4
        self._add(lambda s, d=d, xp=x.t.data_ptr(), yp=y.t.data_ptr(): H.check(self.lib.lt_pwchain_fwd(C.byref(d), xp, yp, s), "lt_pwchain_fwd"),
                  "pwchain", label, flops, nbytes, {"specs": specs, "x": x, "y": y})
        return y

    def can_bottleneck(self, x, convs, strides):
        if not self._fusable() or len(convs) != 3:
            return False
        return bool(H.lib().lt_sel_bottleneck(self.code, H.dims(x.shape), (H.WShape * 3)(*map(H.wshape, convs)), H.i3(strides)))

    def bottleneck(self, x, convs, bns):
        assert self.can_bottleneck(x, convs, (1, 1, 1))
        return self._bneck(x, convs, bns)

    def _bneck(self, x, convs, bns, down=None):
        N, _, Hh, W, Cin = x.shape
        P, Cc = convs[0].shape[0], convs[2].shape[0]
        y = self.alloc((N, 1, Hh, W, Cc))
        if down is None:
            d = H.BneckDesc()
            d.dtype, d.N, d.H, d.W, d.C, d.P = self.code, N, Hh, W, Cc, P
        else:
            d = H.BneckDsDesc()
            d.dtype, d.N, d.H, d.W, d.Cin, d.P, d.C = self.code, N, Hh, W, Cin, P, Cc
        flops0, specs, shape = self.flops, [], x.shape
        for i, (w, bn) in enumerate(zip(convs, bns)):
            spec, d.weight[i], d.scale[i], d.shift[i] = self._pack_layer(w, bn, shape, 1 if i == 1 else 0, H.EPI_RELU_POST)
            specs.append(spec)
            shape = (N, 1, Hh, W, spec.Cout)
        if down is not None:
            spec, d.weight[3], d.scale[3], d.shift[3] = self._pack_layer(*down, x.shape, 0, 0)
            specs.append(spec)
        self.keep += [x.t, d]
        flops = self.flops - flops0
        esz = x.t.element_size()
        nbytes = (x.t.numel() + y.t.numel()) * esz + sum(sp.phases[0].weight.numel() for sp in specs) * esz
        name, fwd = ("bneck", "lt_bottleneck_fwd") if down is None else ("bneck-ds", "lt_bottleneck_ds_fwd")
        label = "%s %d->%d->%d @%s" % (name, Cin, P, Cc, "x".join(str(v) for v in (N, 1, Hh, W)))
        self._add(lambda s, d=d, xp=x.t.data_ptr(), yp=y.t.data_ptr(): H.check(getattr(self.lib, fwd)(C.byref(d), xp, yp, s), fwd),
                  "conv", label, flops, nbytes, {name.replace("-", "_"): True, "specs": specs, "x": x, "y": y})
        return y

    def can_bottleneck_ds(self, x, convs, strides, w_down, stride_down):
        if not self._fusable() or len(convs) != 3:
            return False
        return bool(H.lib().lt_sel_bottleneck_ds(self.code, H.dims(x.shape), (H.WShape * 3)(*map(H.wshape, convs)), H.i3(strides), H.wshape(w_down),
                                                  stride_down))

    def bottleneck_ds(self, x, convs, bns, w_down, bn_down):
        assert self.can_bottleneck_ds(x, convs, (1, 1, 1), w_down, 1)
        return self._bneck(x, convs, bns, (w_down, bn_down))

    def can_expand_reduce(self, t2, res, w_expand, w_reduce):
        if not self._fusable():
            return False
        return bool(H.lib().lt_sel_expand_reduce(self.code, H.dims(t2.shape), H.dims(res.shape), H.wshape(w_expand), H.wshape(w_reduce)))

    def expand_reduce(self, t2, res, w_expand, bn_expand, w_reduce, bn_reduce):
        assert self.can_expand_reduce(t2, res, w_expand, w_reduce)
        N, _, Hh, W, P = t2.shape
        Cc = res.shape[-1]
        y = self.alloc((N, 1, Hh, W, Cc))
        t1 = self.alloc((N, 1, Hh, W, P))
        d = H.XrDesc()
        d.dtype, d.C, d.P, d.M = self.code, Cc, P, N * Hh * W
        flops0 = self.flops
        s3, d.weight[0], d.scale[0], d.shift[0] = self._pack_layer(w_expand, bn_expand, t2.shape, 0, H.EPI_RELU_POST)
        s1, d.weight[1], d.scale[1], d.shift[1] = self._pack_layer(w_reduce, bn_reduce, res.shape, 0, H.EPI_RELU_POST)
        packed = self.const(torch.cat([s3.scale, s3.shift, s1.scale, s1.shift]))
        d.consts = packed.data_ptr()
        self.keep += [t2.t, res.t, d]
        flops = self.flops - flops0
        esz = t2.t.element_size()
        nbytes = (t2.t.numel() + res.t.numel() + y.t.numel() + t1.t.numel() + 2 * Cc * P) * esz
        label = "xr expand %d->%d + reduce %d->%d @%s" % (P, Cc, Cc, P, "x".join(str(v) for v in (N, 1, Hh, W)))
        self._add(lambda s, d=d, a=t2.t.data_ptr(), r=res.t.data_ptr(), yp=y.t.data_ptr(), tp=t1.t.data_ptr():
                  H.check(self.lib.lt_expand_reduce_fwd(C.byref(d), a, r, yp, tp, s), "lt_expand_reduce_fwd"),
                  "conv", label, flops, nbytes, {"xr": True, "specs": [s3, s1], "x": t2, "res": res, "y": y, "t1": t1})
        return y, t1

    def can_stem_pool(self, x, weight, stride, pad, pool):
        return bool(H.lib().lt_sel_stem_pool(self.code, H.dims(x.shape), H.wshape(weight), stride, pad, H.i3(pool)))

    def stem_pool(self, x, weight, bn, image_cell=None):
        assert self.can_stem_pool(x, weight, 2, 3, (3, 2, 1))
        if self.dry_run or weight.shape[1] != 3:
            image_cell = None
        assert image_cell is None or not self.ops, "an op reading the caller's tensor must be the first of the plan"
        N, _, Hh, W, _ = x.shape
        spec = make_conv_spec(weight, None, bn, x.shape, 2, 3, self.dtype, False, H.EPI_RELU_POST)
        Hp, Wp = (spec.Ho - 1) // 2 + 1, (spec.Wo - 1) // 2 + 1
        y = self.alloc((N, 1, Hp, Wp, 64))
        wdev = self.const(spec.phases[0].weight, self.dtype)
        bi, sc, sh = self.const(spec.bias), self.const(spec.scale), self.const(spec.shift)
        wpk = torch.empty(57344 if self.dry_run else self.lib.lt_stem_packed_bytes(), dtype=torch.uint8, device=self.device)
        if not self.dry_run:
            H.check(self.lib.lt_stem_pack_weights(wdev.data_ptr(), spec.k_pad, wpk.data_ptr(), H.cur_stream()), "lt_stem_pack_weights")
            torch.cuda.current_stream().synchronize()
        d = H.StemDesc()
        d.dtype, d.N, d.H, d.W, d.Cin, d.Cout = self.code, N, Hh, W, (3 if image_cell is not None else 8), 64
        d.weight, d.bias, d.scale, d.shift = wpk.data_ptr(), bi.data_ptr(), sc.data_ptr(), sh.data_ptr()
        d.x_layout = 1 if image_cell is not None else 0
        self.keep.append(x.t)
        self.keep.append(d)
        self.keep.append(wpk)
        flops = 2 * N * spec.Ho * spec.Wo * 64 * 49 * weight.shape[1]
        self.flops += flops
        esz = x.t.element_size()
        if image_cell is not None:
            def launch(s, d=d, yp=y.t.data_ptr(), cell=image_cell):
                if not cell.get("ptr"):
                    raise RuntimeError("stem_pool: the plan reads the caller's images; set image_cell['ptr'] before Plan.run")
                H.check(self.lib.lt_stem_pool_fwd(C.byref(d), cell["ptr"], yp, s), "lt_stem_pool_fwd")
            nbytes = N * 3 * Hh * W * 4 + y.t.numel() * esz + spec.phases[0].weight.numel() * esz
            self.npre += 1
        else:
            def launch(s, d=d, xp=x.t.data_ptr(), yp=y.t.data_ptr()):
                H.check(self.lib.lt_stem_pool_fwd(C.byref(d), xp, yp, s), "lt_stem_pool_fwd")
            nbytes = (x.t.numel() + y.t.numel()) * esz + spec.phases[0].weight.numel() * esz
        self._add(launch, "stem", "stem conv7x7/2+pool3x3/2 %d->64 @%s" % (d.Cin, "x".join(str(v) for v in (N, Hh, W))), flops, nbytes,
                  {"spec": spec, "x": x, "y": y})
        return y

    def maxpool(self, x, k, s, p, nd):
        N, D, Hh, W, Cc = x.shape
        kk = (1, k, k) if nd == 2 else (k, k, k)
        ss = (1, s, s) if nd == 2 else (s, s, s)
        pp = (0, p, p) if nd == 2 else (p, p, p)
        od = [(dim + 2 * pp[i] - kk[i]) // ss[i] + 1 for i, dim in enumerate((D, Hh, W))]
        y = self.alloc((N, od[0], od[1], od[2], Cc))
        self.keep.append(x.t)
        self._add(lambda st, xp=x.t.data_ptr(), yp=y.t.data_ptr(), a=(N, D, Hh, W, Cc), kk=H.i3(kk), ss=H.i3(ss), pp=H.i3(pp):
                  H.check(self.lib.lt_maxpool_fwd(self.code, xp, yp, a[0], a[1], a[2], a[3], a[4], kk, ss, pp, st), "lt_maxpool_fwd"),
                  "maxpool", "maxpool%dd k%d @%s" % (nd, k, "x".join(map(str, x.shape))), 0,
                  (x.t.numel() + y.t.numel()) * x.t.element_size(), {"x": x, "y": y, "k": kk, "s": ss, "p": pp})
# ... 118 lines not shown
```

### learnable-triangulation-pytorch_amd/lt_hip.py

```python
import ctypes as C
import os

import torch

HERE = os.path.dirname(os.path.abspath(__file__))
LIB_PATH = os.environ.get("LT_HIP_LIB") or os.path.join(HERE, "lib", "liblt_hip.so")

LT_F32, LT_BF16, LT_FP8 = 0, 1, 2
AGG = {"sum": 0, "max": 1, "softmax": 2, "conf": 3, "conf_norm": 4}
LT_MODEL_ALG, LT_MODEL_RANSAC = 1, 2
LT_KIND_MPII, LT_KIND_COCO = 0, 1
KIND = {"mpii": LT_KIND_MPII, "coco": LT_KIND_COCO}
EPI_RELU_PRE, EPI_RELU_POST, EPI_STORE_F32, EPI_SIGMOID = 1, 2, 4, 8
EPI_RES_F32 = 64
BN_FROZEN = 32
BN_Y_BF16 = 128
ACT_BF16 = 256
TILE_AUTO, TILE_128x128, TILE_128x64, TILE_256x32, TILE_256x16, TILE_64x64, TILE_DIRECT = 0, 1, 2, 3, 4, 5, 99
TILE2_128x128, TILE2_128x64, TILE2_256x32, TILE2_256x16, TILE2_64x64 = 11, 12, 13, 14, 15
TILE_HALO = 20
TILE3_288 = 30
MAX_PHASES = 8

vp, i32, i64, f32, f64 = C.c_void_p, C.c_int32, C.c_int64, C.c_float, C.c_double


class ConvPhase(C.Structure):
    _fields_ = [("weight", vp), ("taps", vp), ("ntaps", i32), ("out_off", i32 * 3), ("weight_frag", vp), ("weight_frag_layout", i32)]


class ConvDesc(C.Structure):
    _fields_ = [("dtype", i32), ("N", i32), ("D", i32), ("H", i32), ("W", i32), ("Cin", i32),
                ("Do", i32), ("Ho", i32), ("Wo", i32), ("stride", i32 * 3), ("pad", i32 * 3),
                ("OD", i32), ("OH", i32), ("OW", i32), ("out_stride", i32 * 3),
                ("Cout", i32), ("ldc", i32), ("cout_pad", i32), ("k_pad", i32),
                ("nphase", i32), ("flags", i32), ("tile", i32), ("stages", i32),
                ("phase", ConvPhase * MAX_PHASES)]


class ConvSkip(C.Structure):
    _fields_ = [("x", vp), ("cin", i32), ("weight_frag", vp)]


class ConvCat2(C.Structure):
    _fields_ = [("x", vp), ("cin", i32), ("H", i32), ("W", i32), ("stride", i32)]


class WShape(C.Structure):
    _fields_ = [("nd", i32), ("s", i64 * 5)]


def wshape(t):
    return WShape(t.dim(), (i64 * 5)(*t.shape))


def dims(shape):
    return (i32 * 5)(*shape)


PWCHAIN_MAX = 3


class PwChainDesc(C.Structure):
    _fields_ = [("dtype", i32), ("nlayers", i32), ("rows", i64), ("cin", i32), ("ldy", i32),
                ("cout", i32 * PWCHAIN_MAX), ("k_pad", i32 * PWCHAIN_MAX), ("flags", i32 * PWCHAIN_MAX),
                ("weight", vp * PWCHAIN_MAX), ("bias", vp * PWCHAIN_MAX), ("scale", vp * PWCHAIN_MAX), ("shift", vp * PWCHAIN_MAX),
                ("plane", i64)]


class StemDesc(C.Structure):
    _fields_ = [("dtype", i32), ("N", i32), ("H", i32), ("W", i32), ("Cin", i32), ("Cout", i32),
                ("weight", vp), ("bias", vp), ("scale", vp), ("shift", vp), ("x_layout", i32)]


class BneckDesc(C.Structure):
    _fields_ = [("dtype", i32), ("N", i32), ("H", i32), ("W", i32), ("C", i32), ("P", i32),
                ("weight", vp * 3), ("bias", vp * 3), ("scale", vp * 3), ("shift", vp * 3)]


class BneckDsDesc(C.Structure):
    _fields_ = [("dtype", i32), ("N", i32), ("H", i32), ("W", i32), ("Cin", i32), ("P", i32), ("C", i32),
                ("weight", vp * 4), ("scale", vp * 4), ("shift", vp * 4)]


class XrDesc(C.Structure):
    _fields_ = [("dtype", i32), ("C", i32), ("P", i32), ("M", C.c_int64), ("weight", vp * 2), ("scale", vp * 2), ("shift", vp * 2), ("consts", vp)]


class NamedTensor(C.Structure):
    _fields_ = [("name", C.c_char_p), ("data", vp), ("ndim", i32), ("shape", C.c_int64 * 5)]


class VolPlanConfig(C.Structure):
    _fields_ = [("dtype", i32), ("num_layers", i32), ("style_caffe", i32), ("num_joints", i32), ("B", i32), ("NV", i32), ("H", i32), ("W", i32),
                ("volume_size", i32), ("cuboid_side", C.c_double), ("volume_multiplier", C.c_double), ("volume_softmax", i32), ("aggregation", i32),
                ("transfer_cmu_to_human36m", i32), ("use_graph", i32)]


class AlgPlanConfig(C.Structure):
    _fields_ = [("model", i32), ("dtype", i32), ("num_layers", i32), ("style_caffe", i32), ("num_joints", i32), ("B", i32), ("NV", i32), ("H", i32),
                ("W", i32), ("use_confidences", i32), ("heatmap_softmax", i32), ("heatmap_multiplier", C.c_double), ("direct_optimization", i32),
                ("reprojection_error_epsilon", C.c_double), ("use_graph", i32)]


class CascadePlanConfig(C.Structure):
    _fields_ = [("alg", AlgPlanConfig), ("vol", VolPlanConfig), ("kind", i32)]


class PlanInfo(C.Structure):
    _fields_ = [("launches", i32), ("heatmap_h", i32), ("heatmap_w", i32), ("flops", C.c_double), ("bytes_allocated", C.c_int64),
                ("n_expand_reduce", i32), ("n_bottleneck", i32), ("n_bottleneck_ds", i32), ("n_conv_cat2", i32), ("n_conv2d_halo", i32), ("n_pwchain", i32),
                ("n_stem_pool", i32), ("n_splitk", i32), ("n_conv_skip", i32), ("graph_captured", i32), ("logits", vp), ("logits_planar", i32)]


SIGNATURES = {
    "lt_plan_create_vol": (C.c_int, [C.POINTER(VolPlanConfig), C.POINTER(NamedTensor), i32, C.POINTER(vp)]),
    "lt_plan_forward_vol": (C.c_int, [vp, vp, vp, vp, vp, vp, vp, vp, vp, vp, vp, vp, vp]),
    "lt_plan_create_alg": (C.c_int, [C.POINTER(AlgPlanConfig), C.POINTER(NamedTensor), i32, C.POINTER(vp)]),
    "lt_plan_forward_alg": (C.c_int, [vp, vp, vp, vp, vp, vp, vp, vp]),
    "lt_plan_create_cascade": (C.c_int, [C.POINTER(CascadePlanConfig), C.POINTER(NamedTensor), i32, C.POINTER(NamedTensor), i32, C.POINTER(vp)]),
    "lt_plan_forward_cascade": (C.c_int, [vp, vp, vp, vp, vp, vp, vp, vp, vp, vp, vp, vp, vp, vp]),
    "lt_plan_set_view_mask": (C.c_int, [vp, vp]),
    "lt_plan_info": (C.c_int, [vp, C.POINTER(PlanInfo)]),
    "lt_plan_destroy": (None, [vp]),
    "lt_last_error": (C.c_char_p, []),
    "lt_abi_version": (C.c_int, []),
    "lt_device_info": (C.c_int, [C.POINTER(C.c_int), C.POINTER(C.c_int), C.c_char_p, C.c_int]),
    "lt_conv_fwd": (C.c_int, [C.POINTER(ConvDesc), vp, vp, vp, vp, vp, vp, vp]),
    "lt_conv_skip_fwd": (C.c_int, [C.POINTER(ConvDesc), vp, vp, vp, vp, C.POINTER(ConvSkip), vp, vp]),
    "lt_conv_cat2_fwd": (C.c_int, [C.POINTER(ConvDesc), vp, C.POINTER(ConvCat2), vp, vp, vp, vp, vp, vp]),
    "lt_conv_cout_pad": (C.c_int, [i32]),
    "lt_conv_chunk_samples": (i32, [i32, i64]),
    "lt_sel_conv_skip": (C.c_int, [i32, i32 * 5, C.POINTER(WShape), i32 * 5, C.POINTER(WShape)]),
    "lt_sel_conv_cat2": (C.c_int, [i32, i32 * 5, C.POINTER(WShape), i32 * 5, C.POINTER(WShape), i32]),
    "lt_sel_splitk_slices": (C.c_int, [C.POINTER(ConvDesc), C.POINTER(WShape), i32]),
    "lt_sel_bottleneck": (C.c_int, [i32, i32 * 5, WShape * 3, i32 * 3]),
    "lt_sel_bottleneck_ds": (C.c_int, [i32, i32 * 5, WShape * 3, i32 * 3, C.POINTER(WShape), i32]),
    "lt_sel_expand_reduce": (C.c_int, [i32, i32 * 5, i32 * 5, C.POINTER(WShape), C.POINTER(WShape)]),
    "lt_sel_stem_pool": (C.c_int, [i32, i32 * 5, C.POINTER(WShape), i32, i32, i32 * 3]),
    "lt_sel_pwchain": (C.c_int, [i32, i32 * 5, i32, C.POINTER(WShape)]),
    "lt_sel_frag_layout": (C.c_int, [C.POINTER(ConvDesc), C.POINTER(WShape), i32, i32]),
    "lt_conv_pack_weights": (C.c_int, [vp, i32, i32, vp, vp]),
    "lt_conv_pack_weights_t32": (C.c_int, [vp, i32, i32, i32, i32, vp, vp]),
    "lt_conv_pack_weights32": (C.c_int, [vp, i32, i32, vp, vp]),
    "lt_pwchain_fwd": (C.c_int, [C.POINTER(PwChainDesc), vp, vp, vp]),
    "lt_stem_pool_fwd": (C.c_int, [C.POINTER(StemDesc), vp, vp, vp]),
    "lt_bottleneck_fwd": (C.c_int, [C.POINTER(BneckDesc), vp, vp, vp]),
    "lt_bottleneck_ds_fwd": (C.c_int, [C.POINTER(BneckDsDesc), vp, vp, vp]),
    "lt_expand_reduce_fwd": (C.c_int, [C.POINTER(XrDesc), vp, vp, vp, vp, vp]),
    "lt_stem_packed_bytes": (C.c_size_t, []),
    "lt_stem_pack_weights": (C.c_int, [vp, i32, vp, vp]),
    "lt_maxpool_fwd": (C.c_int, [i32, vp, vp, i32, i32, i32, i32, i32, i32 * 3, i32 * 3, i32 * 3, vp]),
    "lt_global_avgpool": (C.c_int, [i32, vp, vp, i32, i32, i32, vp]),
    "lt_nchw_to_nhwc": (C.c_int, [i32, vp, vp, i32, i32, i32, i32, vp]),
    "lt_nhwc_to_nchw_f32": (C.c_int, [i32, vp, vp, i32, i32, i32, i32, vp]),
    "lt_coord_volumes": (C.c_int, [vp, vp, vp, f32, i32, i32, i32, vp, vp]),
    "lt_rotate_points": (C.c_int, [vp, vp, vp, i64, vp]),
    "lt_unproject_fwd": (C.c_int, [i32, vp, vp, vp, vp, vp, i32, i32, i32, i32, i32, i32, i32, i32, i32, vp]),
    "lt_unproject_grid_fwd": (C.c_int, [i32, vp, vp, vp, vp, vp, f32, i32, vp, vp, vp, i32, i32, i32, i32, i32, i32, i32, vp]),
    "lt_unproject_masked_fwd": (C.c_int, [i32, vp, vp, vp, vp, vp, vp, i32, i32, i32, i32, i32, i32, i32, i32, i32, vp]),
    "lt_unproject_grid_masked_fwd": (C.c_int, [i32, vp, vp, vp, vp, vp, f32, i32, vp, vp, vp, vp, i32, i32, i32, i32, i32, i32, i32, vp]),
    "lt_cuboid_from_keypoints": (C.c_int, [vp, i32, i32, i32, C.c_double, vp, vp, vp]),
    "lt_softargmax3d_workspace": (C.c_size_t, [i32, i32, i64]),
    "lt_softargmax3d_fwd": (C.c_int, [vp, vp, f32, i32, i32, i32, vp, vp, i32, i32, i64, vp, vp]),
    "lt_softargmax2d_fwd": (C.c_int, [vp, f32, i32, vp, vp, i32, i32, i32, vp]),
    "lt_triangulate_dlt": (C.c_int, [vp, vp, vp, vp, i32, i32, i32, vp]),
    "lt_alg_tail_fwd": (C.c_int, [vp, vp, i32, vp, f32, f32, vp, vp, vp, i32, i32, i32, vp]),
    "lt_alg_tail_masked_fwd": (C.c_int, [vp, vp, i32, vp, f32, f32, vp, vp, vp, vp, i32, i32, i32, vp]),
    "lt_heatmap_argmax_nchw_f32": (C.c_int, [vp, i32, vp, vp, vp, i32, i32, i32, i32, i32, i32, vp]),
    "lt_triangulate_ransac": (C.c_int, [vp, vp, vp, i32, C.c_double, i32, vp, vp, i32, i32, i32, vp]),
    "lt_crop_resize_u8": (C.c_int, [vp, i64, vp, vp, i32, i32, i32, vp, vp, vp]),
    "lt_undistort_crop_resize_u8": (C.c_int, [vp, i64, vp, vp, vp, i64, i32, i32, i32, vp, vp, vp]),
    "lt_bn_act_fwd": (C.c_int, [vp, vp, vp, vp, vp, vp, vp, vp, i64, i32, f32, i32, vp]),
    "lt_bn_act_bwd_workspace": (C.c_size_t, [i64, i32]),
    "lt_bn_act_bwd": (C.c_int, [vp, vp, vp, vp, vp, vp, vp, vp, vp, vp, vp, vp, i32, i64, i32, f32, i32, vp, vp]),
    "lt_act_bwd": (C.c_int, [vp, vp, vp, vp, vp, i32, i64, i32, vp]),
    "lt_channel_sum_workspace": (C.c_size_t, [i64, i32]),
    "lt_channel_sum": (C.c_int, [vp, i64, i32, vp, i32, vp, vp]),
    "lt_channel_sum_dt": (C.c_int, [i32, vp, i64, i32, vp, i32, vp, vp]),
    "lt_maxpool_bwd_dt": (C.c_int, [i32, vp, vp, vp, i32, i32, i32, i32, i32, i32 * 3, i32 * 3, i32 * 3, vp]),
    "lt_convert_pad": (C.c_int, [i32, vp, i32, vp, i64, i32, i32, vp]),
    "lt_maxpool_bwd": (C.c_int, [vp, vp, vp, i32, i32, i32, i32, i32, i32 * 3, i32 * 3, i32 * 3, vp]),
    "lt_adam_step_multi": (C.c_int, [vp, i32, i32, f64, f64, f32, f32, i32, vp]),
    "lt_add_f32": (C.c_int, [vp, vp, i64, vp]),
    "lt_pad_channels_f32": (C.c_int, [vp, vp, i64, i32, i32, vp]),
    "lt_zero": (C.c_int, [vp, i64, vp]),
    "lt_softargmax2d_bwd": (C.c_int, [vp, vp, vp, C.c_float, i32, vp, i32, i32, i32, vp]),
    "lt_triangulate_dlt_bwd": (C.c_int, [vp, vp, vp, vp, vp, vp, i32, i32, i32, vp]),
    "lt_splitk_reduce": (C.c_int, [i32, vp, i32, i64, i64, i32, vp, vp, vp, vp, vp, i32, vp]),
    "lt_add_i64_multi": (C.c_int, [vp, i32, i64, vp]),
    "lt_cast_f32_bf16": (C.c_int, [vp, vp, i64, vp]),
    "lt_gather_f32_multi": (C.c_int, [vp, i32, i32, vp]),
    "lt_amax_f32": (C.c_int, [vp, i64, vp, vp]),
    "lt_amax_dt": (C.c_int, [i32, vp, i64, vp, vp]),
    "lt_quant_fp8_dt": (C.c_int, [i32, vp, vp, i64, vp, vp, vp]),
    "lt_quant_fp8": (C.c_int, [vp, vp, i64, vp, vp, vp]),
    "lt_gather_f32_fp8": (C.c_int, [vp, vp, vp, i64, vp, vp, vp]),
    "lt_scale_product": (C.c_int, [vp, i32, vp, vp, vp]),
    "lt_gather_f32": (C.c_int, [vp, vp, vp, i64, vp]),
    "lt_gather_f32_bf16": (C.c_int, [vp, vp, vp, i64, vp]),
    "lt_conv_wgrad_workspace": (C.c_size_t, [i64, i32, i32]),
    "lt_pack_n8_bf16_bytes": (C.c_size_t, [i32, i64, i32]),
    "lt_pack_n8_bf16": (C.c_int, [vp, vp, i32, i64, i32, i32, vp]),
    "lt_pack_n8_from_bf16": (C.c_int, [vp, vp, i32, i64, i32, i32, vp]),
    "lt_conv_wgrad_bf16_workspace": (C.c_size_t, [i64, i32, i32]),
    "lt_conv_wgrad_bf16": (C.c_int, [vp, vp, vp, vp, i32, i32, i32, i32, i32, i32, i32, i32, i32 * 3, i32 * 3, i32, i32, i32, i32, i32, i32, vp, vp]),
    "lt_conv_wgrad_bf16_nhwc_ok": (C.c_int, [i32, i32, i32, i32, i32, i32, i32, i32, i32, i32 * 3, i32 * 3, i32, i32, i32, i32, i32]),
    "lt_conv_wgrad_bf16_nhwc": (C.c_int, [vp, vp, vp, vp, i32, i32, i32, i32, i32, i32, i32, i32, i32, i32 * 3, i32 * 3, i32, i32, i32, i32, i32, i32, vp, vp]),
    "lt_conv_wgrad": (C.c_int, [vp, vp, vp, vp, i32, i32, i32, i32, i32, i32, i32, i32, i32 * 3, i32 * 3, i32, i32, i32, i32, i32, i32, vp, vp]),
    "lt_adam_step": (C.c_int, [vp, vp, vp, vp, i64, f32, f64, f64, f32, f32, i32, vp]),
    "lt_unproject_bwd_workspace": (C.c_size_t, [i32, i32, i32, i32, i32, i32]),
    "lt_unproject_bwd": (C.c_int, [i32, vp, vp, vp, vp, vp, vp, vp, i32, i32, i32, i32, i32, i32, i32, i32, i32, vp, C.c_size_t, vp]),
    "lt_global_avgpool_bwd": (C.c_int, [vp, vp, i32, i32, i32, i32, vp]),
    "lt_global_avgpool_bwd_dt": (C.c_int, [i32, vp, vp, i32, i32, i32, i32, vp]),
    "lt_softargmax3d_bwd": (C.c_int, [vp, vp, vp, vp, vp, vp, f32, i32, i32, vp, i32, i32, i64, vp]),
    "lt_softargmax3d_bwd_dense": (C.c_int, [vp, vp, vp, vp, vp, vp, vp, vp, f32, i32, i32, vp, i32, i32, i64, vp]),
    "lt_volumetric_ce_fwd": (C.c_int, [vp, vp, vp, vp, vp, vp, vp, i32, i32, i64, vp]),
    "lt_bn_stats_workspace": (C.c_size_t, [i64, i32]),
    "lt_bn_stats_fwd": (C.c_int, [i32, vp, i64, i32, vp, vp, vp, vp, f32, vp, vp]),
    "lt_graph_begin": (C.c_int, [vp]),
    "lt_graph_end": (C.c_int, [vp, C.POINTER(vp)]),
    "lt_graph_launch": (C.c_int, [vp, vp]),
    "lt_graph_destroy": (C.c_int, [vp]),
    "lt_event_create": (C.c_int, [C.POINTER(vp)]),
    "lt_event_record": (C.c_int, [vp, vp]),
    "lt_event_elapsed_ms": (C.c_int, [vp, vp, C.POINTER(f32)]),
    "lt_event_destroy": (C.c_int, [vp]),
}

_lib = None

# ... 106 lines not shown
```

### learnable-triangulation-pytorch_amd/mvn/models/pose_resnet.py

```python
import torch
import torch.nn as nn

import lt_engine as E
import lt_hip as H

BN_MOMENTUM = 0.1

resnet_spec = {18: ("basic", [2, 2, 2, 2]), 34: ("basic", [3, 4, 6, 3]), 50: ("bottleneck", [3, 4, 6, 3]),
               101: ("bottleneck", [3, 4, 23, 3]), 152: ("bottleneck", [3, 8, 36, 3])}


def _bn(c):
    return nn.BatchNorm2d(c, momentum=BN_MOMENTUM)


def bn_tuple(bn):
    return E.BnParams(bn)


class ResidualBlock(nn.Module):

    def __init__(self, kind, inplanes, planes, stride=1, downsample=None, caffe=False):
        super().__init__()
        self.kind, self.stride = kind, stride
        if kind == "bottleneck":
            s1, s2 = (stride, 1) if caffe else (1, stride)
            shapes = [(inplanes, planes, 1, s1), (planes, planes, 3, s2), (planes, planes * 4, 1, 1)]
        else:
            shapes = [(inplanes, planes, 3, stride), (planes, planes, 3, 1)]
        self.strides = [s for _, _, _, s in shapes]
        for i, (ci, co, k, s) in enumerate(shapes, 1):
            setattr(self, "conv%d" % i, nn.Conv2d(ci, co, k, s, k // 2, bias=False))
            setattr(self, "bn%d" % i, _bn(co))
        self.downsample = downsample

    expansion = property(lambda self: 4 if self.kind == "bottleneck" else 1)

    def is_identity_bottleneck(self):
        return self.kind == "bottleneck" and self.downsample is None and all(s == 1 for s in self.strides)

    def record(self, b, x, t1=None, next_block=None):
        n = len(self.strides)
        if self.kind == "bottleneck" and self.downsample is None and t1 is None and next_block is None:
            convs = [self.conv1.weight, self.conv2.weight, self.conv3.weight]
            if b.can_bottleneck(x, convs, self.strides):
                return b.bottleneck(x, convs, [bn_tuple(self.bn1), bn_tuple(self.bn2), bn_tuple(self.bn3)])
        if self.kind == "bottleneck" and self.downsample is not None and t1 is None and next_block is None:
            convs = [self.conv1.weight, self.conv2.weight, self.conv3.weight]
            if b.can_bottleneck_ds(x, convs, self.strides, self.downsample[0].weight, self.downsample[0].stride[0]):
                return b.bottleneck_ds(x, convs, [bn_tuple(self.bn1), bn_tuple(self.bn2), bn_tuple(self.bn3)], self.downsample[0].weight,
                                       bn_tuple(self.downsample[1]))
        if t1 is not None or next_block is not None:
            assert self.is_identity_bottleneck()
            if t1 is None:
                t1 = b.conv(x, self.conv1.weight, None, bn_tuple(self.bn1), stride=1, pad=0, relu=True)
            t2 = b.conv(t1, self.conv2.weight, None, bn_tuple(self.bn2), stride=1, pad=1, relu=True)
            b.release(t1)
            if next_block is not None and b.can_expand_reduce(t2, x, self.conv3.weight, next_block.conv1.weight):
                y, t1n = b.expand_reduce(t2, x, self.conv3.weight, bn_tuple(self.bn3), next_block.conv1.weight, bn_tuple(next_block.bn1))
                b.release(t2)
                return y, t1n
            y = b.conv(t2, self.conv3.weight, None, bn_tuple(self.bn3), stride=1, pad=0, relu=True, residual=x)
            b.release(t2)
            return (y, None) if next_block is not None else y
        if self.kind == "bottleneck" and self.downsample is not None:
            ds, sds = self.downsample[0], self.downsample[0].stride[0]
            Ho, Wo = (x.shape[2] - 1) // sds + 1, (x.shape[3] - 1) // sds + 1
            if b.can_conv_cat2((x.shape[0], 1, Ho, Wo, self.conv3.weight.shape[1]), self.conv3.weight, x.shape, ds.weight, sds):
                t1 = b.conv(x, self.conv1.weight, None, bn_tuple(self.bn1), stride=self.conv1.stride[0], pad=0, relu=True)
                t2 = b.conv(t1, self.conv2.weight, None, bn_tuple(self.bn2), stride=self.conv2.stride[0], pad=1, relu=True)
                b.release(t1)
                y = b.conv_cat2(t2, self.conv3.weight, bn_tuple(self.bn3), x, ds.weight, bn_tuple(self.downsample[1]), sds)
                b.release(t2)
                return y
        res = x
        if self.downsample is not None:
            res = b.conv(x, self.downsample[0].weight, None, bn_tuple(self.downsample[1]), stride=self.downsample[0].stride[0], pad=0)
        y = x
        for i in range(1, n + 1):
            conv, bn = getattr(self, "conv%d" % i), getattr(self, "bn%d" % i)
            last = i == n
            z = b.conv(y, conv.weight, None, bn_tuple(bn), stride=conv.stride[0], pad=conv.padding[0], relu=True,
                       residual=res if last else None)
            if y is not x:
                b.release(y)
            y = z
        if res is not x:
            b.release(res)
        return y


class GlobalAveragePoolingHead(nn.Module):

    def __init__(self, in_channels, n_classes):
        super().__init__()
        self.features = nn.Sequential(
            nn.Conv2d(in_channels, 512, 3, stride=1, padding=1), _bn(512), nn.MaxPool2d(2), nn.ReLU(inplace=True),
            nn.Conv2d(512, 256, 3, stride=1, padding=1), _bn(256), nn.MaxPool2d(2), nn.ReLU(inplace=True))
        self.head = nn.Sequential(nn.Linear(256, 512), nn.ReLU(inplace=True), nn.Linear(512, 256), nn.ReLU(inplace=True),
                                  nn.Linear(256, n_classes), nn.Sigmoid())

    def record(self, b, x):
        f = self.features
        y = b.conv(x, f[0].weight, f[0].bias, bn_tuple(f[1]), stride=1, pad=1, relu=True)
        p = b.maxpool(y, 2, 2, 0, nd=2); b.release(y)
        y = b.conv(p, f[4].weight, f[4].bias, bn_tuple(f[5]), stride=1, pad=1, relu=True); b.release(p)
        p = b.maxpool(y, 2, 2, 0, nd=2); b.release(y)
        g = b.global_avgpool(p); b.release(p)
        h = self.head
        y = b.conv(g, h[0].weight[:, :, None, None], h[0].bias, None, relu=True); b.release(g)
        z = b.conv(y, h[2].weight[:, :, None, None], h[2].bias, None, relu=True); b.release(y)
        o = b.conv(z, h[4].weight[:, :, None, None], h[4].bias, None, sigmoid=True, out_f32=True); b.release(z)
        return o


class PoseResNet(E.PlanCache):
    def __init__(self, block_kind, layers, num_joints, num_input_channels=3, deconv_with_bias=False, num_deconv_layers=3,
                 num_deconv_filters=(256, 256, 256), num_deconv_kernels=(4, 4, 4), final_conv_kernel=1,
                 alg_confidences=False, vol_confidences=False, caffe=False):
        super().__init__()
        assert all(k == 4 for k in num_deconv_kernels), "only the 4x4 stride-2 deconvolution of the reference configs"
        self.num_joints, self.num_input_channels = num_joints, num_input_channels
        self.block_kind, self.caffe = block_kind, caffe
        exp = 4 if block_kind == "bottleneck" else 1
        self.conv1 = nn.Conv2d(num_input_channels, 64, kernel_size=7, stride=2, padding=3, bias=False)
        self.bn1 = _bn(64)
        inplanes = 64
        for li, (planes, nb) in enumerate(zip((64, 128, 256, 512), layers), 1):
            stride = 1 if li == 1 else 2
            blocks = []
            for bi in range(nb):
                st = stride if bi == 0 else 1
                ds = None
                if bi == 0 and (st != 1 or inplanes != planes * exp):
                    ds = nn.Sequential(nn.Conv2d(inplanes, planes * exp, kernel_size=1, stride=st, bias=False), _bn(planes * exp))
                blocks.append(ResidualBlock(block_kind, inplanes, planes, st, ds, caffe))
                inplanes = planes * exp
            setattr(self, "layer%d" % li, nn.Sequential(*blocks))
        if alg_confidences:
            self.alg_confidences = GlobalAveragePoolingHead(inplanes, num_joints)
        if vol_confidences:
            self.vol_confidences = GlobalAveragePoolingHead(inplanes, 32)
        dl = []
        for i in range(num_deconv_layers):
            dl += [nn.ConvTranspose2d(inplanes, num_deconv_filters[i], kernel_size=4, stride=2, padding=1, output_padding=0,
                                      bias=deconv_with_bias), _bn(num_deconv_filters[i]), nn.ReLU(inplace=True)]
            inplanes = num_deconv_filters[i]
        self.deconv_layers = nn.Sequential(*dl)
        self.final_layer = nn.Conv2d(inplanes, num_joints, kernel_size=final_conv_kernel, stride=1,
                                     padding=1 if final_conv_kernel == 3 else 0)
        self.compute_dtype = torch.float32
        self._init_plan_cache()

    def record(self, b, x, want_heatmaps=True, image_cell=None):
        if b.can_stem_pool(x, self.conv1.weight, 2, 3, (3, 2, 1)):
            y = b.stem_pool(x, self.conv1.weight, bn_tuple(self.bn1), image_cell=image_cell)
        else:
            y = b.conv(x, self.conv1.weight, None, bn_tuple(self.bn1), stride=2, pad=3, relu=True)
            p = b.maxpool(y, 3, 2, 1, nd=2); b.release(y)
            y = p
        for li in range(1, 5):
            blocks = list(getattr(self, "layer%d" % li))
            t1 = None
            for bi, blk in enumerate(blocks):
                nxt = blocks[bi + 1] if bi + 1 < len(blocks) else None
                chain = (nxt is not None and blk.is_identity_bottleneck() and nxt.is_identity_bottleneck() and
                         tuple(blk.conv3.weight.shape[:2]) == (1024, 256) and tuple(nxt.conv1.weight.shape[:2]) == (256, 1024) and b.dtype == torch.bfloat16 and
                         not b.live_weights)
                if chain:
                    z, t1n = blk.record(b, y, t1=t1, next_block=nxt)
                elif t1 is not None:
                    z, t1n = blk.record(b, y, t1=t1), None
                else:
                    z, t1n = blk.record(b, y), None
                b.release(y)
                y, t1 = z, t1n
        alg = self.alg_confidences.record(b, y) if hasattr(self, "alg_confidences") else None
        vol = self.vol_confidences.record(b, y) if hasattr(self, "vol_confidences") else None
        for i in range(0, len(self.deconv_layers), 3):
            dc, bn = self.deconv_layers[i], self.deconv_layers[i + 1]
            z = b.conv(y, dc.weight, dc.bias, bn_tuple(bn), stride=2, pad=1, transposed=True, relu=True)
            b.release(y)
            y = z
        feats = y
        hm = None
        if want_heatmaps:
            fl = self.final_layer
            hm = b.conv(feats, fl.weight, fl.bias, None, stride=1, pad=fl.padding[0], out_f32=True)
        return hm, feats, alg, vol

    def heatmap_shape(self, h, w):
        def down(v, k, s, p):
            return (v + 2 * p - k) // s + 1
        for k, s, p in ((7, 2, 3), (3, 2, 1), (3, 2, 1), (3, 2, 1), (3, 2, 1)):
            h, w = down(h, k, s, p), down(w, k, s, p)
        return h * 8, w * 8

    def forward(self, x):
        H.require_gpu(x, "images")
        if self.training:
            raise NotImplementedError("training runs through VolumetricTriangulationNet, whose step is recorded as a whole (lt_train.py); "
                                      "the stand-alone forward of this module is inference only: call .eval()")
        key = (tuple(x.shape), self.compute_dtype, x.device)
        N, _, Hh, W = x.shape

        def build():
            b = E.PlanBuilder(x.device, self.compute_dtype)
            inp = b.alloc((N, 1, Hh, W, E.min_cin_of(self.compute_dtype)))
            outs = self.record(b, inp, True)
            return {"plan": b.finish(), "inp": inp, "outs": outs}

        with torch.cuda.device(x.device):
            P = self._plan_for(key, build)
            plan, inp, (hm, feats, alg, vol) = P["plan"], P["inp"], P["outs"]
            st = torch.cuda.current_stream(x.device).cuda_stream
            E.stage_images(x.float().contiguous(), inp, st)
            plan.run_eager(st)
            to_nchw = lambda a: a.t[:, 0].permute(0, 3, 1, 2).to(torch.float32, copy=True)
            conf = lambda a: None if a is None else a.t.reshape(N, -1).clone()
            return to_nchw(hm), to_nchw(feats), conf(alg), conf(vol)


def get_pose_net(config, device="cuda:0"):
    kind, layers = resnet_spec[config.num_layers]
    if config.style == "caffe":
        kind = "bottleneck"
    model = PoseResNet(kind, layers, config.num_joints, num_input_channels=3, deconv_with_bias=False, num_deconv_layers=3,
                       num_deconv_filters=(256, 256, 256), num_deconv_kernels=(4, 4, 4), final_conv_kernel=1,
                       alg_confidences=config.alg_confidences, vol_confidences=config.vol_confidences,
                       caffe=(config.style == "caffe"))
    if config.init_weights:
        print("Loading pretrained weights from: {}".format(config.checkpoint))
        own = model.state_dict()
        loaded = torch.load(config.checkpoint, map_location="cpu")
        loaded = loaded.get("state_dict", loaded)
        picked = {}
        for k, v in loaded.items():
            name = k.replace("module.", "")
            if name in own and v.shape == own[name].shape:
                picked[name] = v
            elif name in ("final_layer.weight", "final_layer.bias"):
                print("Reiniting final layer:", k)
                o = torch.zeros_like(own[name])
                if name.endswith("weight"):
                    nn.init.xavier_uniform_(o)
                n = min(o.shape[0], v.shape[0])
                o[:n] = v[:n]
                picked[name] = o
# ... 7 lines not shown
```

Before: 1430 samples/s.

## Fuse layer1's last bottleneck with layer2's first 1x1 reduce conv

Adds a TAIL variant of the bottleneck kernel. After computing the block output, it also runs the next stage's first 1x1 reduce (256->128) from an LDS chunk buffer and writes t1 for the next block, optionally storing y at stride 2. The downsample block then consumes that t1 plus a conv_cat2 for the expand and downsample. This removes a separate conv launch and a reread of the 256-channel activation from global memory. In exchange the kernel does more MFMA work and needs more LDS and registers, which may hurt occupancy or scheduling.

```diff
diff --git a/include/lt_hip.h b/include/lt_hip.h
--- a/include/lt_hip.h
+++ b/include/lt_hip.h
@@ -98,6 +98,7 @@
 int lt_sel_splitk_slices(const lt_conv_desc* d, const lt_wshape* w, int32_t transposed);
 int lt_sel_bottleneck(int32_t dtype, const int32_t x[5], const lt_wshape w[3], const int32_t strides[3]);
 int lt_sel_bottleneck_ds(int32_t dtype, const int32_t x[5], const lt_wshape w[3], const int32_t strides[3], const lt_wshape* w_down, int32_t stride_down);
+int lt_sel_bottleneck_reduce(int32_t dtype, const int32_t x[5], const lt_wshape w[3], const int32_t strides[3], const lt_wshape* w_next, int32_t stride_down);
 int lt_sel_expand_reduce(int32_t dtype, const int32_t t2[5], const int32_t res[5], const lt_wshape* w_expand, const lt_wshape* w_reduce);
 int lt_sel_stem_pool(int32_t dtype, const int32_t x[5], const lt_wshape* w, int32_t stride, int32_t pad, const int32_t pool[3]);
 int lt_sel_pwchain(int32_t dtype, const int32_t x[5], int32_t nlayers, const lt_wshape* w);
@@ -290,6 +291,22 @@
 
 typedef struct {
     int32_t dtype;
+    int32_t N, H, W;
+    int32_t C, P, P_next;
+    int32_t out_stride;
+    const void* weight[3];
+    const float* bias[3];
+    const float* scale[3];
+    const float* shift[3];
+    const void* weight_next;
+    const float* bias_next;
+    const float* scale_next;
+    const float* shift_next;
+} lt_bneck_reduce_desc;
+int lt_bottleneck_reduce_fwd(const lt_bneck_reduce_desc* desc, const void* x, void* y, void* t1_next, void* stream);
+
+typedef struct {
+    int32_t dtype;
     int32_t C, P;
     int64_t M;
     const void* weight[2];
diff --git a/learnable-triangulation-pytorch_amd/csrc/bneck.hip b/learnable-triangulation-pytorch_amd/csrc/bneck.hip
--- a/learnable-triangulation-pytorch_amd/csrc/bneck.hip
+++ b/learnable-triangulation-pytorch_amd/csrc/bneck.hip
@@ -33,6 +33,14 @@
     int N, H, W, tiles_x, tiles_y;
 };
 
+struct BneckTailArgs : BneckArgs {
+    const bf16_t* w4;
+    bf16_t* t1n;
+    const float* bias4;
+    const float* scale4;
+    const float* shift4;
+};
+
 template <int NK1, int AHEAD, int D>
 constexpr int bneck_after(int ks) {
     int total = 0, last = 0;
@@ -45,8 +53,8 @@
     return total - last;
 }
 
-template <int C, int P, int NSTR, int NHELD>
-__global__ __launch_bounds__(256, 2) void bneck_kernel(const BneckArgs a) {
+template <int C, int P, int NSTR, int NHELD, int TAIL = 0>
+__global__ __launch_bounds__(256, 2) void bneck_kernel(const std::conditional_t<TAIL != 0, BneckTailArgs, BneckArgs> a) {
     typedef bf16_t T;
     constexpr int TH = 8, TW = 16, HPI = TW + 2, HROWS = (TH + 2) * HPI;
     constexpr int NPB = 4;
@@ -248,15 +256,24 @@
     __syncthreads();
     BN_STAMP(2);
 
-    constexpr int NU3 = NOBW * G2, WD3 = G2 < 6 ? G2 : 6;
+    constexpr int PN = 128, G4 = TAIL != 0 ? PN / 16 : 0, NUQ = G2 + G4;
+    constexpr int NU3 = NOBW * NUQ, WD3 = G2 < 6 ? G2 : 6;
     int poff[NPB];
 #pragma unroll
     for (int pb = 0; pb < NPB; ++pb)
         poff[pb] = ((img * a.H + ty * TH + 2 * pb + prr) * a.W + tx * TW + pcc) * C + 8 * hk;
     const T* wl3 = a.w3 + (size_t)lane * 8;
+    const T* wl4 = nullptr;
+    if constexpr (TAIL != 0) wl4 = a.w4 + (size_t)lane * 8;
     auto load_w3 = [&](int u) -> V16 {
-        const int q = u / G2, g = u - q * G2;
+        const int q = u / NUQ, g = u - q * NUQ;
         V16 v;
+        if constexpr (TAIL != 0) {
+            if (g >= G2) {
+                v.u = *(const uint4*)(wl4 + ((size_t)(G4 * q + g - G2) * (PN / 32) + wave) * 512);
+                return v;
+            }
+        }
         v.u = *(const uint4*)(wl3 + ((size_t)g * NOB + wave + 4 * q) * 512);
         return v;
     };
@@ -347,7 +364,127 @@
     __syncthreads();
     BN_STAMP(4);
 
-    {
+    if constexpr (TAIL != 0) {
+        constexpr int RB4 = 2 * PN, CH_OFF = T2_OFF + NPB * 32 * RB;
+        static_assert(C == 256 && P == 64 && (TAIL == 1 || TAIL == 2), "the last block of ResNet layer1");
+        static_assert(CH_OFF % 256 == 0 && CH_OFF + NPB * 32 * RB4 <= 80 * 1024, "chunk buffer: alignment of the XOR argument, two workgroups per CU");
+        const unsigned a2 = lds0 + T2_OFF + n31 * RB + ((hk ^ fsw(n31)) << 4);
+        const unsigned a4 = lds0 + CH_OFF + n31 * RB4 + ((hk ^ (n31 & 15)) << 4);
+        const bool st = TAIL == 1 || (prr == 0 && (n31 & 1) == 0);
+        int yoff[NPB];
+#pragma unroll
+        for (int pb = 0; pb < NPB; ++pb)
+            yoff[pb] = TAIL == 1 ? ((img * a.H + ty * TH + 2 * pb + prr) * a.W + tx * TW + pcc) * C + 8 * hk
+                                 : ((img * (a.H >> 1) + ty * (TH / 2) + pb) * (a.W >> 1) + tx * (TW / 2) + (pcc >> 1)) * C + 8 * hk;
+        f32x16 acc[NPB], acc4[NPB];
+        float4 c4s[4], c4f[4];
+        static_for<0, NU3>([&](auto uc) {
+            constexpr int u = decltype(uc)::value;
+            constexpr int q = u / NUQ, g = u % NUQ;
+            const int ob = wave + 4 * q;
+            if constexpr (g == 0) {
+#pragma unroll
+                for (int pb = 0; pb < NPB; ++pb)
+#pragma unroll
+                    for (int e = 0; e < 16; ++e) acc[pb][e] = 0.f;
+            }
+            if constexpr (g == G2 - WD3 && q + 1 < NOBW && q + 1 > NHELD) load_res(q + 1, rq[(q + 1 - NHELD) & 1]);
+            if constexpr (u + WD3 < NU3) wf3[(u + WD3) % (WD3 + 1)] = load_w3(u + WD3);
+            V16 xb[NPB];
+            if constexpr (g < G2) {
+#pragma unroll
+                for (int pb = 0; pb < NPB; ++pb) xb[pb].u = *(const uint4*)((lptr_t)(size_t)((a2 ^ (g << 5)) + pb * 32 * RB));
+#pragma unroll
+                for (int pb = 0; pb < NPB; ++pb)
+                    acc[pb] = __builtin_amdgcn_mfma_f32_32x32x16_bf16(wf3[u % (WD3 + 1)].h, xb[pb].h, acc[pb], 0, 0, 0);
+                __builtin_amdgcn_sched_barrier(0);
+            } else {
+                constexpr int g4 = g - G2;
+                if constexpr (q == 0 && g4 == 0) {
+#pragma unroll
+                    for (int pb = 0; pb < NPB; ++pb)
+#pragma unroll
+                        for (int e = 0; e < 16; ++e) acc4[pb][e] = 0.f;
+                }
+                if constexpr (q == NOBW - 1 && g4 == 0) {
+#pragma unroll
+                    for (int i = 0; i < 4; ++i) {
+                        const int c = 32 * wave + 16 * (i >> 1) + 8 * hk + 4 * (i & 1);
+                        c4s[i] = *(const float4*)(a.scale4 + c);
+                        c4f[i] = *(const float4*)(a.shift4 + c);
+                    }
+                }
+#pragma unroll
+                for (int pb = 0; pb < NPB; ++pb) xb[pb].u = *(const uint4*)((lptr_t)(size_t)((a4 ^ (g4 << 5)) + pb * 32 * RB4));
+#pragma unroll
+                for (int pb = 0; pb < NPB; ++pb)
+                    acc4[pb] = __builtin_amdgcn_mfma_f32_32x32x16_bf16(wf3[u % (WD3 + 1)].h, xb[pb].h, acc4[pb], 0, 0, 0);
+                __builtin_amdgcn_sched_barrier(0);
+            }
+            if constexpr (g == G2 - 1) {
+                if constexpr (q > 0) asm volatile("s_waitcnt lgkmcnt(0)\n\ts_barrier" ::: "memory");
+#pragma unroll
+                for (int j = 0; j < 2; ++j) {
+                    float esc[8], esf[8];
+#pragma unroll
+                    for (int e = 0; e < 8; ++e) {
+                        esc[e] = csel(cst3, 64 * q, 8 * j + e);
+                        esf[e] = csel(cst3, 64 * q + 32, 8 * j + e);
+                    }
+                    if (a.bias[2]) {
+#pragma unroll
+                        for (int e = 0; e < 8; ++e) esf[e] = a.bias[2][32 * ob + 16 * j + 8 * hk + e] * esc[e] + esf[e];
+                    }
+                    unsigned o[NPB][4];
+#pragma unroll
+                    for (int pb = 0; pb < NPB; ++pb) {
+                        uint4 rv;
+                        if constexpr (q < NHELD) rv = held[q < NHELD ? q : 0][pb][j];
+                        else rv = rq[(q - NHELD) & 1][pb][j];
+                        const unsigned rr[4] = {rv.x, rv.y, rv.z, rv.w};
+#pragma unroll
+                        for (int d = 0; d < 4; ++d) {
+                            const int e = 2 * d;
+                            const float v0 = fmaxf(acc[pb][8 * j + e] * esc[e] + esf[e] + __uint_as_float(rr[d] << 16), 0.f);
+                            const float v1 = fmaxf(acc[pb][8 * j + e + 1] * esc[e + 1] + esf[e + 1] + __uint_as_float(rr[d] & 0xffff0000u), 0.f);
+                            o[pb][d] = pack_bf16x2(v0, v1);
+                        }
+                        const int slot = (4 * wave + 2 * j + hk) ^ (n31 & 15);
+                        *(uint4*)((lptr_t)(size_t)(lds0 + CH_OFF + (32 * pb + n31) * RB4 + slot * 16)) = make_uint4(o[pb][0], o[pb][1], o[pb][2], o[pb][3]);
+                    }
+                    if (st) {
+#pragma unroll
+                        for (int pb = 0; pb < NPB; ++pb)
+                            *(uint4*)(a.y + yoff[pb] + 32 * ob + 16 * j) = make_uint4(o[pb][0], o[pb][1], o[pb][2], o[pb][3]);
+                    }
+                }
+                asm volatile("s_waitcnt lgkmcnt(0)\n\ts_barrier" ::: "memory");
+            }
+        });
+        BN_STAMP(6);
+        float esc[16], esf[16], ebi[16];
+#pragma unroll
+        for (int i = 0; i < 4; ++i) {
+            esc[4 * i] = c4s[i].x; esc[4 * i + 1] = c4s[i].y; esc[4 * i + 2] = c4s[i].z; esc[4 * i + 3] = c4s[i].w;
+            esf[4 * i] = c4f[i].x; esf[4 * i + 1] = c4f[i].y; esf[4 * i + 2] = c4f[i].z; esf[4 * i + 3] = c4f[i].w;
+        }
+#pragma unroll
+        for (int e = 0; e < 16; ++e) ebi[e] = a.bias4 ? a.bias4[32 * wave + 16 * (e >> 3) + 8 * hk + (e & 7)] : 0.f;
+#pragma unroll
+        for (int pb = 0; pb < NPB; ++pb) {
+            bf16_t* tp = a.t1n + ((size_t)((img * a.H + ty * TH + 2 * pb + prr) * a.W + tx * TW + pcc) * PN + 32 * wave + 8 * hk);
+#pragma unroll
+            for (int q2 = 0; q2 < 2; ++q2) {
+                unsigned o[4];
+#pragma unroll
+                for (int d = 0; d < 4; ++d) {
+                    const int e = 8 * q2 + 2 * d;
+                    o[d] = pack_bf16x2(fmaxf((acc4[pb][e] + ebi[e]) * esc[e] + esf[e], 0.f), fmaxf((acc4[pb][e + 1] + ebi[e + 1]) * esc[e + 1] + esf[e + 1], 0.f));
+                }
+                *(uint4*)(tp + 16 * q2) = make_uint4(o[0], o[1], o[2], o[3]);
+            }
+        }
+    } else {
         const unsigned a2 = lds0 + T2_OFF + n31 * RB + ((hk ^ fsw(n31)) << 4);
         f32x16 acc[NPB];
         static_for<0, NU3>([&](auto uc) {
@@ -403,6 +540,18 @@
         });
     }
     BN_STAMP(5);
+}
+
+template <int NHELD, int OS>
+int launch_bneck_tail(const BneckTailArgs& a, hipStream_t s) {
+    constexpr int lds = 180 * 128 + 128 * 128 + 128 * 256;
+    static_assert(lds <= 80 * 1024 && lds >= 180 * 128 + 3 * 180 * 64 + 192 * 64, "two workgroups per CU; phase 1's ring");
+    auto kern = bneck_kernel<256, 64, 4, NHELD, OS>;
+    LT_OPT_IN_LDS(kern, lds);
+    const long long nblk = (long long)a.N * a.tiles_x * a.tiles_y;
+    hipLaunchKernelGGL(kern, dim3((unsigned)nblk), dim3(256), lds, s, a);
+    LT_CHECK_LAUNCH("lt_bottleneck_reduce_fwd");
+    return LT_OK;
 }
 
 template <int C, int P, int NSTR, int NHELD>
@@ -774,6 +923,44 @@
     return launch_bneck<512, 128, 3, LT_BNECK_HELD128>(a, s);
 }
 
+#ifndef LT_BNECK_HELD_TAIL
+#define LT_BNECK_HELD_TAIL 2
+#endif
+extern "C" int lt_bottleneck_reduce_fwd(const lt_bneck_reduce_desc* d, const void* x, void* y, void* t1_next, void* stream) {
+    LT_REQUIRE(d && x && y && t1_next, LT_ERR_INVALID, "lt_bottleneck_reduce_fwd: null argument");
+    LT_REQUIRE(x != y && x != t1_next && y != t1_next, LT_ERR_INVALID, "lt_bottleneck_reduce_fwd: the outputs must not alias the input or each other");
+    LT_REQUIRE(d->dtype == LT_BF16, LT_ERR_UNSUPPORTED, "lt_bottleneck_reduce_fwd: bf16 only");
+    LT_REQUIRE(d->C == 256 && d->P == 64 && d->P_next == 128, LT_ERR_UNSUPPORTED,
+               "lt_bottleneck_reduce_fwd: widths %d / %d -> %d (256 / 64 -> 128: the last block of ResNet layer1 and layer2's first reduce)", d->C, d->P, d->P_next);
+    LT_REQUIRE(d->out_stride == 1 || d->out_stride == 2, LT_ERR_UNSUPPORTED, "lt_bottleneck_reduce_fwd: out_stride %d (1 or 2)", d->out_stride);
+    LT_REQUIRE(d->N > 0 && d->H > 0 && d->W > 0 && d->H % 8 == 0 && d->W % 16 == 0, LT_ERR_UNSUPPORTED,
+               "lt_bottleneck_reduce_fwd: map %d x %d (8 x 16 pixel tiles)", d->H, d->W);
+    LT_REQUIRE((long long)d->N * d->H * d->W * d->C < (1ll << 31), LT_ERR_UNSUPPORTED, "lt_bottleneck_reduce_fwd: 32-bit element offsets");
+    BneckTailArgs a;
+    a.x = (const bf16_t*)x;
+    a.y = (bf16_t*)y;
+    a.w1 = (const bf16_t*)d->weight[0];
+    a.w2 = (const bf16_t*)d->weight[1];
+    a.w3 = (const bf16_t*)d->weight[2];
+    for (int i = 0; i < 3; ++i) {
+        LT_REQUIRE(d->weight[i] && d->scale[i] && d->shift[i], LT_ERR_INVALID, "lt_bottleneck_reduce_fwd: layer %d: null weight / scale / shift", i);
+        a.bias[i] = d->bias[i];
+        a.scale[i] = d->scale[i];
+        a.shift[i] = d->shift[i];
+    }
+    LT_REQUIRE(d->weight_next && d->scale_next && d->shift_next, LT_ERR_INVALID, "lt_bottleneck_reduce_fwd: the reduce: null weight / scale / shift");
+    a.w4 = (const bf16_t*)d->weight_next;
+    a.t1n = (bf16_t*)t1_next;
+    a.bias4 = d->bias_next;
+    a.scale4 = d->scale_next;
+    a.shift4 = d->shift_next;
+    a.N = d->N; a.H = d->H; a.W = d->W;
+    a.tiles_x = d->W / 16; a.tiles_y = d->H / 8;
+    hipStream_t s = (hipStream_t)stream;
+    if (d->out_stride == 2) return launch_bneck_tail<LT_BNECK_HELD_TAIL, 2>(a, s);
+    return launch_bneck_tail<LT_BNECK_HELD_TAIL, 1>(a, s);
+}
+
 extern "C" int lt_bottleneck_ds_fwd(const lt_bneck_ds_desc* d, const void* x, void* y, void* stream) {
     LT_REQUIRE(d && x && y, LT_ERR_INVALID, "lt_bottleneck_ds_fwd: null argument");
     LT_REQUIRE(x != y, LT_ERR_INVALID, "lt_bottleneck_ds_fwd: in-place is not possible");
diff --git a/learnable-triangulation-pytorch_amd/csrc/plan.hip b/learnable-triangulation-pytorch_amd/csrc/plan.hip
--- a/learnable-triangulation-pytorch_amd/csrc/plan.hip
+++ b/learnable-triangulation-pytorch_amd/csrc/plan.hip
@@ -248,6 +248,7 @@
     std::deque<lt_stem_desc> stem_descs;
     std::deque<lt_bneck_desc> bneck_descs;
     std::deque<lt_bneck_ds_desc> bneck_ds_descs;
+    std::deque<lt_bneck_reduce_desc> bneck_reduce_descs;
     std::deque<lt_xr_desc> xr_descs;
     hipGraphExec_t graph = nullptr;
     bool captured = false;
@@ -581,6 +582,27 @@
         ++n_bneck;
         return LT_OK;
     }
+    int bottleneck_reduce(const Act& x, const WT w[3], const BN bn[3], const WT& wn, const BN& bnn, int sds, Act& y, Act& t1) {
+        const int Pn = (int)wn.s[0];
+        PL_TRY(alloc(x.n, 1, x.h / sds, x.w / sds, x.c, es, y));
+        PL_TRY(alloc(x.n, 1, x.h, x.w, Pn, es, t1));
+        bneck_reduce_descs.emplace_back();
+        lt_bneck_reduce_desc& d = bneck_reduce_descs.back();
+        memset(&d, 0, sizeof(d));
+        d.dtype = dtype; d.N = x.n; d.H = x.h; d.W = x.w; d.C = x.c; d.P = (int)w[0].s[0]; d.P_next = Pn; d.out_stride = sds;
+        int shape[5] = {x.n, 1, x.h, x.w, x.c};
+        for (int i = 0; i < 3; ++i) {
+            ConvSpec sp;
+            PL_TRY(pack_block_layer(w[i], bn[i], shape, i == 1 ? 1 : 0, LT_EPI_RELU_POST, &d.weight[i], &d.scale[i], &d.shift[i], sp));
+            shape[4] = sp.Cout;
+        }
+        ConvSpec sp;
+        PL_TRY(pack_block_layer(wn, bnn, shape, 0, LT_EPI_RELU_POST, &d.weight_next, &d.scale_next, &d.shift_next, sp));
+        const lt_bneck_reduce_desc* dp = &d; const void* xp = x.p; void* yp = y.p; void* tp = t1.p;
+        ops.push_back([=](hipStream_t s) { return lt_bottleneck_reduce_fwd(dp, xp, yp, tp, s); });
+        ++n_bneck;
+        return LT_OK;
+    }
     int bottleneck_ds(const Act& x, const WT w[3], const BN bn[3], const WT& wd, const BN& bnd, Act& y) {
         const int Cc = (int)w[2].s[0];
         PL_TRY(alloc(x.n, 1, x.h, x.w, Cc, es, y));
@@ -662,9 +684,29 @@
         if (ds) { PL_TRY(get(pre + ".downsample.0.weight", b.wd, 4)); PL_TRY(get_bn(pre + ".downsample.1", (int)b.wd.s[0], b.bnd)); }
         return LT_OK;
     }
-    int record_block(const Block& b, const Act& x, const Act* t1_in, const Block* nxt, Act& y, Act& t1n) {
+    int reduce_behind(const Block& nf, const Act& x, const lt_wshape w3[3], const int strides[3]) {
+        if (!nf.bottleneck || !nf.has_ds || nf.strides[0] != 1) return 0;
+        const int sds = nf.sds;
+        const lt_wshape wn = wshape(nf.w[0]), we = wshape(nf.w[2]), wd = wshape(nf.wd);
+        if (nf.strides[1] != sds || x.h % sds || x.w % sds || !lt_sel_bottleneck_reduce(dtype, dims(x).data(), w3, strides, &wn, sds)) return 0;
+        const int t2s[5] = {x.n, 1, x.h / sds, x.w / sds, (int)nf.w[2].s[1]}, xs[5] = {x.n, 1, x.h / sds, x.w / sds, x.c};
+        return lt_sel_conv_cat2(dtype, t2s, &we, xs, &wd, 1) ? sds : 0;
+    }
+    int record_block(const Block& b, const Act& x, const Act* t1_in, const Block* nxt, Act& y, Act& t1n, const Block* nstage = nullptr) {
         t1n = Act();
         const lt_wshape w3[3] = {wshape(b.w[0]), wshape(b.w[1]), wshape(b.w[2])}, wd = wshape(b.wd);
+        if (t1_in && b.has_ds) {
+            Act t2; ConvOpt o;
+            o.bn = &b.bn[1]; o.relu = true; o.stride = b.strides[1]; o.pad = 1; PL_TRY(conv(*t1_in, b.w[1], o, t2));
+            release(*t1_in);
+            PL_TRY(conv_cat2(t2, b.w[2], b.bn[2], x, b.wd, b.bnd, 1, y));
+            release(t2);
+            return LT_OK;
+        }
+        if (nstage && b.identity_bottleneck() && !t1_in && !nxt) {
+            const int sds = reduce_behind(*nstage, x, w3, b.strides);
+            if (sds) return bottleneck_reduce(x, b.w, b.bn, nstage->w[0], nstage->bn[0], sds, y, t1n);
+        }
         if (b.bottleneck && !b.has_ds && !t1_in && !nxt && lt_sel_bottleneck(dtype, dims(x).data(), w3, b.strides)) return bottleneck(x, b.w, b.bn, y);
         if (b.bottleneck && b.has_ds && !t1_in && !nxt && lt_sel_bottleneck_ds(dtype, dims(x).data(), w3, b.strides, &wd, b.sds))
             return bottleneck_ds(x, b.w, b.bn, b.wd, b.bnd, y);
@@ -767,19 +809,30 @@
         }
         int inplanes = 64;
         const int planes_of[4] = {64, 128, 256, 512};
+        std::vector<Block> stage[4];
         for (int li = 0; li < 4; ++li) {
             const int planes = planes_of[li], stride = li == 0 ? 1 : 2;
-            std::vector<Block> blocks(nb[li]);
+            stage[li].resize(nb[li]);
             for (int bi = 0; bi < nb[li]; ++bi) {
                 const int st = bi == 0 ? stride : 1;
                 const bool ds = bi == 0 && (st != 1 || inplanes != planes * exp);
-                PL_TRY(load_block("backbone.layer" + std::to_string(li + 1) + "." + std::to_string(bi), bott, caffe, st, ds, blocks[bi]));
+                PL_TRY(load_block("backbone.layer" + std::to_string(li + 1) + "." + std::to_string(bi), bott, caffe, st, ds, stage[li][bi]));
                 inplanes = planes * exp;
             }
-            Act t1; bool have_t1 = false;
+        }
+        Act t1; bool have_t1 = false;
+        for (int li = 0; li < 4; ++li) {
+            const std::vector<Block>& blocks = stage[li];
             for (int bi = 0; bi < nb[li]; ++bi) {
                 const Block& blk = blocks[bi];
                 const Block* nxt = bi + 1 < nb[li] ? &blocks[bi + 1] : nullptr;
+                if (!nxt && li < 3 && !have_t1 && blk.identity_bottleneck()) {
+                    Act z, t1n;
+                    PL_TRY(record_block(blk, y, nullptr, nullptr, z, t1n, &stage[li + 1][0]));
+                    release(y);
+                    y = z; t1 = t1n; have_t1 = !t1n.null();
+                    continue;
+                }
                 const bool chain = nxt && blk.identity_bottleneck() && nxt->identity_bottleneck() && dtype == LT_BF16 && blk.w[2].s[0] == 1024 && blk.w[2].s[1] == 256 &&
                                    nxt->w[0].s[0] == 256 && nxt->w[0].s[1] == 1024;
                 Act z, t1n;
diff --git a/learnable-triangulation-pytorch_amd/csrc/select.hip b/learnable-triangulation-pytorch_amd/csrc/select.hip
--- a/learnable-triangulation-pytorch_amd/csrc/select.hip
+++ b/learnable-triangulation-pytorch_amd/csrc/select.hip
@@ -65,6 +65,12 @@
     return x[2] % 8 == 0 && x[3] % 16 == 0 && (long long)x[0] * x[2] * x[3] * C < (1ll << 31);
 }
 
+extern "C" int lt_sel_bottleneck_reduce(int32_t dtype, const int32_t x[5], const lt_wshape w[3], const int32_t strides[3], const lt_wshape* wn, int32_t sd) {
+    if (env_on("LT_NO_BNECK_TAIL") || !lt_sel_bottleneck(dtype, x, w, strides)) return 0;
+    if (x[4] != 256 || !wshape_is(wn, 4, 128, 256, 1, 1) || (sd != 1 && sd != 2)) return 0;
+    return x[2] % 2 == 0 && x[3] % 2 == 0;
+}
+
 extern "C" int lt_sel_bottleneck_ds(int32_t dtype, const int32_t x[5], const lt_wshape w[3], const int32_t strides[3], const lt_wshape* wd, int32_t sd) {
     if (dtype != LT_BF16 || env_on("LT_NO_BNECK") || env_on("LT_NO_BNECK_DS")) return 0;
     if (x[1] != 1 || strides[0] != 1 || strides[1] != 1 || strides[2] != 1 || sd != 1) return 0;
diff --git a/learnable-triangulation-pytorch_amd/lt_engine.py b/learnable-triangulation-pytorch_amd/lt_engine.py
--- a/learnable-triangulation-pytorch_amd/lt_engine.py
+++ b/learnable-triangulation-pytorch_amd/lt_engine.py
@@ -204,7 +204,7 @@
     def _declines(self, *a, **k):
         return False
 
-    can_conv_skip = can_conv_cat2 = can_chain_pointwise = can_bottleneck = can_bottleneck_ds = can_expand_reduce = can_stem_pool = _declines
+    can_conv_skip = can_conv_cat2 = can_chain_pointwise = can_bottleneck = can_bottleneck_ds = can_bottleneck_reduce = can_expand_reduce = can_stem_pool = _declines
 
 
 class PlanBuilder(Recorder):
@@ -564,6 +564,37 @@
         assert self.can_bottleneck_ds(x, convs, (1, 1, 1), w_down, 1)
         return self._bneck(x, convs, bns, (w_down, bn_down))
 
+    def can_bottleneck_reduce(self, x, convs, strides, w_next, stride_down):
+        if not self._fusable() or len(convs) != 3:
+            return False
+        return bool(H.lib().lt_sel_bottleneck_reduce(self.code, H.dims(x.shape), (H.WShape * 3)(*map(H.wshape, convs)), H.i3(strides), H.wshape(w_next),
+                                                      stride_down))
+
+    def bottleneck_reduce(self, x, convs, bns, w_next, bn_next, stride_down):
+        assert self.can_bottleneck_reduce(x, convs, (1, 1, 1), w_next, stride_down)
+        N, _, Hh, W, Cin = x.shape
+        P, Cc, Pn = convs[0].shape[0], convs[2].shape[0], w_next.shape[0]
+        y = self.alloc((N, 1, Hh // stride_down, W // stride_down, Cc))
+        t1 = self.alloc((N, 1, Hh, W, Pn))
+        d = H.BneckReduceDesc()
+        d.dtype, d.N, d.H, d.W, d.C, d.P, d.P_next, d.out_stride = self.code, N, Hh, W, Cc, P, Pn, stride_down
+        flops0, specs, shape = self.flops, [], x.shape
+        for i, (w, bn) in enumerate(zip(convs, bns)):
+            spec, d.weight[i], d.scale[i], d.shift[i] = self._pack_layer(w, bn, shape, 1 if i == 1 else 0, H.EPI_RELU_POST)
+            specs.append(spec)
+            shape = (N, 1, Hh, W, spec.Cout)
+        spec, d.weight_next, d.scale_next, d.shift_next = self._pack_layer(w_next, bn_next, shape, 0, H.EPI_RELU_POST)
+        specs.append(spec)
+        self.keep += [x.t, d]
+        flops = self.flops - flops0
+        esz = x.t.element_size()
+        nbytes = (x.t.numel() + y.t.numel() + t1.t.numel()) * esz + sum(sp.phases[0].weight.numel() for sp in specs) * esz
+        label = "bneck %d->%d->%d + reduce %d->%d @%s (y at stride %d)" % (Cin, P, Cc, Cc, Pn, "x".join(str(v) for v in (N, 1, Hh, W)), stride_down)
+        self._add(lambda s, d=d, xp=x.t.data_ptr(), yp=y.t.data_ptr(), tp=t1.t.data_ptr():
+                  H.check(self.lib.lt_bottleneck_reduce_fwd(C.byref(d), xp, yp, tp, s), "lt_bottleneck_reduce_fwd"),
+                  "conv", label, flops, nbytes, {"bneck_reduce": True, "specs": specs, "x": x, "y": y, "t1": t1, "stride": stride_down})
+        return y, t1
+
     def can_expand_reduce(self, t2, res, w_expand, w_reduce):
         if not self._fusable():
             return False
diff --git a/learnable-triangulation-pytorch_amd/lt_hip.py b/learnable-triangulation-pytorch_amd/lt_hip.py
--- a/learnable-triangulation-pytorch_amd/lt_hip.py
+++ b/learnable-triangulation-pytorch_amd/lt_hip.py
@@ -81,6 +81,12 @@
 class BneckDsDesc(C.Structure):
     _fields_ = [("dtype", i32), ("N", i32), ("H", i32), ("W", i32), ("Cin", i32), ("P", i32), ("C", i32),
                 ("weight", vp * 4), ("scale", vp * 4), ("shift", vp * 4)]
+
+
+class BneckReduceDesc(C.Structure):
+    _fields_ = [("dtype", i32), ("N", i32), ("H", i32), ("W", i32), ("C", i32), ("P", i32), ("P_next", i32), ("out_stride", i32),
+                ("weight", vp * 3), ("bias", vp * 3), ("scale", vp * 3), ("shift", vp * 3),
+                ("weight_next", vp), ("bias_next", vp), ("scale_next", vp), ("shift_next", vp)]
 
 
 class XrDesc(C.Structure):
@@ -136,6 +142,7 @@
     "lt_sel_splitk_slices": (C.c_int, [C.POINTER(ConvDesc), C.POINTER(WShape), i32]),
     "lt_sel_bottleneck": (C.c_int, [i32, i32 * 5, WShape * 3, i32 * 3]),
     "lt_sel_bottleneck_ds": (C.c_int, [i32, i32 * 5, WShape * 3, i32 * 3, C.POINTER(WShape), i32]),
+    "lt_sel_bottleneck_reduce": (C.c_int, [i32, i32 * 5, WShape * 3, i32 * 3, C.POINTER(WShape), i32]),
     "lt_sel_expand_reduce": (C.c_int, [i32, i32 * 5, i32 * 5, C.POINTER(WShape), C.POINTER(WShape)]),
     "lt_sel_stem_pool": (C.c_int, [i32, i32 * 5, C.POINTER(WShape), i32, i32, i32 * 3]),
     "lt_sel_pwchain": (C.c_int, [i32, i32 * 5, i32, C.POINTER(WShape)]),
@@ -147,6 +154,7 @@
     "lt_stem_pool_fwd": (C.c_int, [C.POINTER(StemDesc), vp, vp, vp]),
     "lt_bottleneck_fwd": (C.c_int, [C.POINTER(BneckDesc), vp, vp, vp]),
     "lt_bottleneck_ds_fwd": (C.c_int, [C.POINTER(BneckDsDesc), vp, vp, vp]),
+    "lt_bottleneck_reduce_fwd": (C.c_int, [C.POINTER(BneckReduceDesc), vp, vp, vp, vp]),
     "lt_expand_reduce_fwd": (C.c_int, [C.POINTER(XrDesc), vp, vp, vp, vp, vp]),
     "lt_stem_packed_bytes": (C.c_size_t, []),
     "lt_stem_pack_weights": (C.c_int, [vp, i32, vp, vp]),
diff --git a/learnable-triangulation-pytorch_amd/mvn/models/pose_resnet.py b/learnable-triangulation-pytorch_amd/mvn/models/pose_resnet.py
--- a/learnable-triangulation-pytorch_amd/mvn/models/pose_resnet.py
+++ b/learnable-triangulation-pytorch_amd/mvn/models/pose_resnet.py
@@ -39,10 +39,32 @@
     def is_identity_bottleneck(self):
         return self.kind == "bottleneck" and self.downsample is None and all(s == 1 for s in self.strides)
 
-    def record(self, b, x, t1=None, next_block=None):
+    def reduce_behind(self, b, x, prev_convs, prev_strides):
+        if self.kind != "bottleneck" or self.downsample is None or self.conv1.stride[0] != 1:
+            return 0
+        sds = self.downsample[0].stride[0]
+        N, _, Hh, W, Cc = x.shape
+        if self.conv2.stride[0] != sds or Hh % sds or W % sds or not b.can_bottleneck_reduce(x, prev_convs, prev_strides, self.conv1.weight, sds):
+            return 0
+        small = (N, 1, Hh // sds, W // sds)
+        return sds if b.can_conv_cat2(small + (self.conv3.weight.shape[1],), self.conv3.weight, small + (Cc,), self.downsample[0].weight, 1) else 0
+
+    def record(self, b, x, t1=None, next_block=None, next_stage=None):
         n = len(self.strides)
+        if t1 is not None and self.downsample is not None:
+            t2 = b.conv(t1, self.conv2.weight, None, bn_tuple(self.bn2), stride=self.conv2.stride[0], pad=1, relu=True)
+            b.release(t1)
+            y = b.conv_cat2(t2, self.conv3.weight, bn_tuple(self.bn3), x, self.downsample[0].weight, bn_tuple(self.downsample[1]), 1)
+            b.release(t2)
+            return y
         if self.kind == "bottleneck" and self.downsample is None and t1 is None and next_block is None:
             convs = [self.conv1.weight, self.conv2.weight, self.conv3.weight]
+            if next_stage is not None:
+                sds = next_stage.reduce_behind(b, x, convs, self.strides)
+                if sds:
+                    return b.bottleneck_reduce(x, convs, [bn_tuple(self.bn1), bn_tuple(self.bn2), bn_tuple(self.bn3)], next_stage.conv1.weight,
+                                               bn_tuple(next_stage.bn1), sds)
+                return self.record(b, x), None
             if b.can_bottleneck(x, convs, self.strides):
                 return b.bottleneck(x, convs, [bn_tuple(self.bn1), bn_tuple(self.bn2), bn_tuple(self.bn3)])
         if self.kind == "bottleneck" and self.downsample is not None and t1 is None and next_block is None:
@@ -159,11 +181,16 @@
             y = b.conv(x, self.conv1.weight, None, bn_tuple(self.bn1), stride=2, pad=3, relu=True)
             p = b.maxpool(y, 3, 2, 1, nd=2); b.release(y)
             y = p
+        t1 = None
         for li in range(1, 5):
             blocks = list(getattr(self, "layer%d" % li))
-            t1 = None
             for bi, blk in enumerate(blocks):
                 nxt = blocks[bi + 1] if bi + 1 < len(blocks) else None
+                if nxt is None and li < 4 and t1 is None and blk.is_identity_bottleneck():
+                    z, t1n = blk.record(b, y, next_stage=getattr(self, "layer%d" % (li + 1))[0])
+                    b.release(y)
+                    y, t1 = z, t1n
+                    continue
                 chain = (nxt is not None and blk.is_identity_bottleneck() and nxt.is_identity_bottleneck() and
                          tuple(blk.conv3.weight.shape[:2]) == (1024, 256) and tuple(nxt.conv1.weight.shape[:2]) == (256, 1024) and b.dtype == torch.bfloat16 and
                          not b.live_weights)
```

Measured after the change: 1445 samples/s (median of 6 runs). +1.0%, better.
